# TencentARC/BlobCtrl

Measured on AMD Instinct MI355X. Metric: 512x512_50step_blobctrl_edits_per_sec, higher is better.
Workload: dtype fp16

## Files before the change

blobctrl_amd/_lib.py:

```python
import ctypes as C
import os

_HERE = os.path.dirname(os.path.abspath(__file__))
LIB_PATH = os.environ.get("BLOBCTRL_HIP_LIB") or os.path.join(_HERE, "libblobctrl_hip.so")

A_DENSE, A_CONV3X3 = 0, 1
ACT_NONE, ACT_GELU, ACT_GEGLU, ACT_SILU, ACT_QUICK_GELU = 0, 1, 2, 3, 4
OUT_F16, OUT_F16_T, OUT_F32 = 0, 1, 2
TILE_NAMES = ["auto", "256x128", "128x128_s3", "128x128_s2", "256x64_s2", "256x64_s3", "128x64", "64x64", "halo128x160", "wreg128x160",
              "gw64x128", "gw64x256", "gw64x320", "g256x256"]
TILE_HALO = 8
TILE_WREG = 9
TILE_GW64x128, TILE_GW64x256, TILE_GW64x320 = 10, 11, 12
TILE_G256 = 13
GW_TILES = {TILE_GW64x128: 2, TILE_GW64x256: 4, TILE_GW64x320: 5}


class BcGemm(C.Structure):
    _fields_ = [
        ("A", C.c_void_p), ("A2", C.c_void_p), ("a_mode", C.c_int),
        ("M", C.c_int), ("N", C.c_int), ("K", C.c_int),
        ("lda", C.c_int), ("lda2", C.c_int), ("C1", C.c_int), ("Cin", C.c_int),
        ("Hin", C.c_int), ("Win", C.c_int), ("Hv", C.c_int), ("Wv", C.c_int),
        ("Hout", C.c_int), ("Wout", C.c_int), ("stride", C.c_int), ("conv_nopad_lo", C.c_int),
# ... 130 lines not shown
    "bc_plan_run_timed": (C.c_int, [C.c_void_p, C.c_int, C.c_void_p, C.POINTER(C.c_float)]),
    "bc_plan_run_timed_kernels": (C.c_int, [C.c_void_p, C.c_int, C.c_void_p, C.POINTER(C.c_float), C.POINTER(C.c_float)]),
    "bc_plan_run_marked": (C.c_int, [C.c_void_p, C.c_int, C.POINTER(C.c_void_p), C.c_int, C.POINTER(C.c_int), C.c_int, C.POINTER(C.c_float)]),
    "bc_plan_save": (C.c_int, [C.c_void_p, C.c_char_p, C.c_void_p, C.c_int]),
    "bc_plan_load": (C.c_int, [C.c_char_p, C.POINTER(C.c_void_p)]),
    "bc_plan_buffer": (C.c_int, [C.c_void_p, C.c_char_p, C.POINTER(C.c_void_p), C.POINTER(C.c_longlong)]),
    "bc_graph_begin": (C.c_int, [C.c_void_p]),
    "bc_graph_end": (C.c_int, [C.c_void_p, C.POINTER(C.c_void_p)]),
    "bc_graph_launch": (C.c_int, [C.c_void_p, C.c_void_p]),
    "bc_graph_destroy": (C.c_int, [C.c_void_p]),
    "bc_event_create": (C.c_int, [C.POINTER(C.c_void_p)]),
    "bc_event_create_sync": (C.c_int, [C.POINTER(C.c_void_p)]),
    "bc_stream_wait_event": (C.c_int, [C.c_void_p, C.c_void_p]),
    "bc_event_record": (C.c_int, [C.c_void_p, C.c_void_p]),
    "bc_event_elapsed_ms": (C.c_int, [C.c_void_p, C.c_void_p, C.POINTER(C.c_float)]),
    "bc_event_destroy": (C.c_int, [C.c_void_p]),
}

EXPORTED_SYMBOLS = tuple(_SIGNATURES.keys())

VAE_SIGNATURES = {
    "bc_vae_tile_blend": (C.c_int, [C.c_void_p, C.c_void_p, C.c_void_p, C.c_void_p, C.c_void_p, C.c_int, C.c_int, C.c_int, C.c_int, C.c_int,
                                    C.c_int, C.c_int, C.c_int, C.c_int, C.c_int, C.c_int, C.c_int, C.c_int, C.c_int, C.c_void_p]),
}
VAE_TILE_DECODE, VAE_TILE_ENCODE = 0, 1

REQUEST_SIGNATURES = {
    "bc_assemble_input_requests": (C.c_int, [C.c_void_p, C.c_int, C.c_void_p, C.c_void_p, C.c_void_p, C.c_int, C.c_int, C.c_int,
                                             C.c_int, C.c_int, C.c_int, C.c_int, C.c_void_p, C.c_void_p, C.c_int, C.c_void_p, C.c_void_p]),
    "bc_assemble_input_im2col_requests": (C.c_int, [C.c_void_p, C.c_int, C.c_void_p, C.c_void_p, C.c_int, C.c_int, C.c_int, C.c_int,
                                                    C.c_int, C.c_void_p, C.c_void_p, C.c_int, C.c_void_p, C.c_void_p]),
    "bc_timestep_embedding_rows": (C.c_int, [C.c_void_p, C.c_int, C.c_int, C.c_void_p, C.c_int, C.c_void_p, C.c_void_p]),
    "bc_scheduler_step_requests": (C.c_int, [C.c_void_p, C.c_void_p, C.c_void_p, C.c_void_p, C.c_void_p, C.c_int, C.c_int, C.c_int,
                                             C.c_void_p, C.c_int, C.c_int, C.c_int, C.c_void_p, C.c_int, C.c_void_p]),
}

_ATTN_RELPOS_ARGS = [C.c_void_p] * 4 + [C.c_int] * 11 + [C.c_longlong] * 4 + [C.c_float] + [C.c_void_p] * 3 + [C.c_void_p]
SAM_SIGNATURES = {
    "bc_attention_relpos": (C.c_int, _ATTN_RELPOS_ARGS),
    "bc_window_partition": (C.c_int, [C.c_void_p, C.c_int, C.c_int, C.c_int, C.c_int, C.c_int, C.c_void_p, C.c_void_p]),
    "bc_window_unpartition": (C.c_int, [C.c_void_p, C.c_void_p, C.c_int, C.c_int, C.c_int, C.c_int, C.c_int, C.c_void_p, C.c_void_p]),
    "bc_add_pos": (C.c_int, [C.c_void_p, C.c_void_p, C.c_int, C.c_int, C.c_int, C.c_void_p, C.c_void_p]),
    "bc_add_rows": (C.c_int, [C.c_void_p, C.c_void_p, C.c_int, C.c_int, C.c_int, C.c_void_p, C.c_void_p]),
    "bc_act_rows": (C.c_int, [C.c_void_p, C.c_longlong, C.c_int, C.c_void_p]),
    "bc_bilinear_resize_f32": (C.c_int, [C.c_void_p] + [C.c_int] * 8 + [C.c_float, C.c_void_p, C.c_void_p]),
    "bc_sam_tokens": (C.c_int, [C.c_void_p, C.c_int, C.c_void_p, C.c_void_p, C.c_int, C.c_void_p, C.c_int, C.c_void_p, C.c_void_p, C.c_float,
                                C.c_void_p, C.c_void_p]),
    "bc_sam_masks": (C.c_int, [C.c_void_p, C.c_int, C.c_void_p, C.c_int, C.c_int, C.c_int, C.c_int, C.c_int, C.c_void_p, C.c_void_p]),
}
SAM_BATCH_SIGNATURES = {
    "bc_sam_tokens_batch": (C.c_int, [C.c_void_p, C.c_int, C.c_void_p, C.c_void_p, C.c_int, C.c_int, C.c_void_p, C.c_int, C.c_void_p, C.c_void_p,
                                      C.c_float, C.c_void_p, C.c_void_p]),
    "bc_mask_stats": (C.c_int, [C.c_void_p, C.c_int, C.c_int, C.c_int, C.c_float, C.c_float, C.c_void_p, C.c_void_p, C.c_void_p]),
}
SAM_HOST_SIGNATURES = {"bc_mask_stats_chunks": (C.c_int, [C.c_int, C.c_int])}

_MASK_REMOVE_ARGS = [C.c_void_p, C.c_int, C.c_int, C.c_int, C.c_int, C.c_int, C.c_void_p, C.c_void_p, C.c_void_p]
MASK_SIGNATURES = {
    "bc_mask_label": (C.c_int, [C.c_void_p, C.c_int, C.c_int, C.c_int, C.c_int, C.c_void_p, C.c_void_p]),
    "bc_mask_remove_small": (C.c_int, _MASK_REMOVE_ARGS + [C.c_void_p]),
    "bc_mask_remove_small_phase": (C.c_int, _MASK_REMOVE_ARGS + [C.c_int, C.c_void_p]),
}
MASK_HOLES, MASK_ISLANDS = 0, 1
MASK_REGION_PHASES = 5

EDIT_SIGNATURES = {
    "bc_ellipse_cover": (C.c_int, [C.c_void_p, C.c_int, C.c_int, C.c_int, C.c_void_p, C.c_void_p]),
    "bc_ellipse_paint": (C.c_int, [C.c_void_p, C.c_int, C.c_int, C.c_int, C.c_void_p, C.c_void_p, C.c_int, C.c_void_p]),
    "bc_mask_row_extents": (C.c_int, [C.c_void_p, C.c_int, C.c_int, C.c_int, C.c_void_p, C.c_void_p]),
    "bc_mask_cutout": (C.c_int, [C.c_void_p, C.c_void_p, C.c_void_p, C.c_int, C.c_int, C.c_int, C.c_void_p, C.c_void_p]),
}
EDIT_MAX_DIM = 16384

RESAMPLE_SIGNATURES = {
    "bc_resample_horizontal": (C.c_int, [C.c_void_p, C.c_int, C.c_int, C.c_int, C.c_int, C.c_int, C.c_void_p, C.c_void_p, C.c_int, C.c_int,
                                         C.c_int, C.c_int, C.c_void_p, C.c_void_p]),
    "bc_resample_vertical": (C.c_int, [C.c_void_p, C.c_int, C.c_int, C.c_int, C.c_int, C.c_int, C.c_void_p, C.c_void_p, C.c_int, C.c_int,
                                       C.c_int, C.c_int, C.c_int, C.c_void_p, C.c_void_p, C.c_void_p, C.c_int, C.c_int, C.c_void_p]),
}

_BLUR_ARGS = [C.c_void_p, C.c_int, C.c_int, C.c_int, C.c_int, C.c_int, C.c_int, C.c_void_p, C.c_void_p]
OVERLAY_SIGNATURES = {
    "bc_box_blur3_rows": (C.c_int, _BLUR_ARGS),
    "bc_box_blur3_cols": (C.c_int, _BLUR_ARGS),
    "bc_mask_bounds": (C.c_int, [C.c_void_p, C.c_int, C.c_int, C.c_int, C.c_void_p, C.c_void_p, C.c_void_p]),
    "bc_overlay_composite": (C.c_int, [C.c_void_p, C.c_void_p, C.c_void_p, C.c_int, C.c_int, C.c_int, C.c_int, C.c_int, C.c_int, C.c_int,
                                       C.c_void_p, C.c_void_p]),
}
BLUR_MAX_R = 63

IP_SIGNATURES = {
    "bc_attention_ip": (C.c_int, [C.c_void_p, C.c_void_p, C.c_void_p, C.c_void_p, C.c_int, C.c_int, C.c_int, C.c_int, C.c_int, C.c_int, C.c_int,
                                  C.c_int, C.c_float, C.c_void_p, C.c_void_p]),
}
ATTENTION_IP_MAX_T = 64
IP_PATH_SIGNATURES = {
    "bc_attention_ip_path": (C.c_int, [C.c_int, C.c_int, C.c_int, C.c_int]),
    "bc_attention_ip_with": (C.c_int, [C.c_int] + IP_SIGNATURES["bc_attention_ip"][1]),
}
ATTENTION_IP_SCALAR, ATTENTION_IP_TILES = 0, 1

IP_MASK_SIGNATURES = {
    "bc_attention_ip_masked": (C.c_int, [C.c_void_p, C.c_void_p, C.c_void_p, C.c_void_p, C.c_int, C.c_int, C.c_int, C.c_int, C.c_int, C.c_int,
                                         C.c_int, C.c_int, C.c_int, C.c_float, C.c_void_p, C.c_void_p, C.c_int, C.c_void_p]),
}
IP_MASK_DIRECT_SIGNATURES = {
    "bc_ip_mask_downsample": (C.c_int, [C.c_void_p, C.c_int, C.c_int, C.c_int, C.c_int, C.c_int, C.c_int, C.c_int, C.c_void_p, C.c_int,
                                        C.c_void_p]),
    "bc_attention_ip_masked_path": (C.c_int, [C.c_int] * 5),
    "bc_attention_ip_masked_with": (C.c_int, [C.c_int] + IP_MASK_SIGNATURES["bc_attention_ip_masked"][1]),
}

class BcTinyConvArgs(C.Structure):
    _fields_ = [("x", C.c_void_p), ("w", C.c_void_p), ("bias", C.c_void_p), ("skip", C.c_void_p), ("out", C.c_void_p),
                ("B", C.c_int), ("H", C.c_int), ("W", C.c_int), ("Ci", C.c_int), ("Co", C.c_int),
                ("up", C.c_int), ("relu", C.c_int), ("out_mode", C.c_int)]


TINY_VAE_SIGNATURES = {
    "bc_tiny_conv3x3_flat": (C.c_int, [C.c_void_p] * 5 + [C.c_int] * 8 + [C.c_void_p]),
    "bc_tiny_latents_in": (C.c_int, [C.c_void_p, C.c_int, C.c_int, C.c_int, C.c_void_p, C.c_void_p]),
}
TINY_VAE_DIRECT_SIGNATURES = {"bc_tiny_conv3x3": (C.c_int, [C.POINTER(BcTinyConvArgs), C.c_void_p])}
TINY_OUT_F16, TINY_OUT_IMAGE, TINY_OUT_U8 = 0, 1, 2

PAG_SIGNATURES = {
    "bc_attention_identity": (C.c_int, [C.c_void_p, C.c_void_p, C.c_int, C.c_int, C.c_int, C.c_int, C.c_int, C.c_int, C.c_void_p]),
    "bc_pag_scheduler_step": (C.c_int, [C.c_void_p] * 6 + [C.c_int] * 3 + [C.c_void_p] + [C.c_int] * 3 + [C.c_void_p, C.c_int, C.c_void_p]),
}

OPS = {"bc_gemm": 0, "bc_gn_stats": 1, "bc_gn_finalize": 2, "bc_gn_apply_fused": 3, "bc_gn_apply": 4, "bc_layernorm": 5,
       "bc_attention": 6, "bc_attention_causal": 7, "bc_assemble_input": 8, "bc_timestep_embedding": 9,
       "bc_timestep_embedding_table": 10, "bc_cfg_scheduler_step": 11, "bc_embed_tokens": 12, "bc_softmax_rows": 13,
       "bc_patchify": 14, "bc_add_cls_pos": 15, "bc_silu": 16, "bc_nchw_to_nhwc_f16": 17, "bc_nhwc_to_nchw": 18,
       "bc_gaussian_sample": 19, "bc_rowchain": 22, "bc_assemble_input_im2col": 23, "bc_memset_zero": 24,
       "bc_rowchain_midx": 25, "bc_rowchain_pack_kv": 26, "bc_rowchain_sum": 27, "bc_ctx_fold": 28, "bc_dup_halves": 29,
       "bc_cfg_scheduler_step_noise": 30, "bc_cfg_scheduler_step3": 31,
       "bc_assemble_input_scaled": 32, "bc_assemble_input_im2col_scaled": 33, "bc_scheduler_step_single": 34,
       "bc_timestep_embedding_table_cond": 35, "bc_timestep_embedding_cond": 36, "bc_freeu": 37}
REQUEST_OPS = {"bc_scheduler_step_requests": 38, "bc_assemble_input_requests": 39, "bc_assemble_input_im2col_requests": 40,
               "bc_timestep_embedding_rows": 41}
SAM_OPS = {"bc_attention_relpos": 42, "bc_window_partition": 43, "bc_window_unpartition": 44, "bc_add_pos": 45, "bc_add_rows": 46,
           "bc_act_rows": 47, "bc_bilinear_resize_f32": 48, "bc_sam_tokens": 49, "bc_sam_masks": 50}
SAM_BATCH_OPS = {"bc_sam_tokens_batch": 51, "bc_mask_stats": 52}
IP_OPS = {"bc_attention_ip": 53}
IP_MASK_OPS = {"bc_attention_ip_masked": 55}
_OP_TABLES = (OPS, REQUEST_OPS, SAM_OPS, SAM_BATCH_OPS, IP_OPS)
_OP_TABLES_BEYOND = (IP_MASK_OPS,)
TINY_VAE_OPS = {"bc_tiny_conv3x3_flat": 57, "bc_tiny_latents_in": 58}
_OP_TABLES_TINY_VAE = (TINY_VAE_OPS,)
PAG_OPS = {"bc_attention_identity": 60, "bc_pag_scheduler_step": 61}
_OP_TABLES_PAG = (PAG_OPS,)
OP_SIGNAL, OP_WAIT = 20, 21
CHAIN_IN, CHAIN_MID, CHAIN_OUT, CHAIN_OUT_FF, CHAIN_OUT_TAIL, CHAIN_MIDX, CHAIN_OUT_FFP = 0, 1, 2, 3, 4, 5, 6
GN_TOT_WORDS = 6
_KIND = {C.c_void_p: "p", C.c_int: "i", C.c_float: "f", C.c_longlong: "l", C.c_char_p: "p"}


def op_code(name):
    for table in _OP_TABLES + _OP_TABLES_BEYOND + _OP_TABLES_TINY_VAE + _OP_TABLES_PAG:
        if name in table:
            return table[name]
    raise KeyError(name)


def op_signature(name):
    args = (_SIGNATURES.get(name) or REQUEST_SIGNATURES.get(name) or SAM_SIGNATURES.get(name) or SAM_BATCH_SIGNATURES.get(name) or
            IP_SIGNATURES.get(name) or IP_MASK_SIGNATURES.get(name) or TINY_VAE_SIGNATURES.get(name) or PAG_SIGNATURES[name])[1][:-1]
    return "".join("p" if (a not in _KIND) else _KIND[a] for a in args)


class BcPlanBuffer(C.Structure):
    _fields_ = [("name", C.c_char_p), ("address", C.c_void_p), ("bytes", C.c_longlong), ("host_data", C.c_void_p)]

_lib = None


class BlobCtrlHipError(RuntimeError):
    pass


def load():
    global _lib
    if _lib is not None:
        return _lib
    if not os.path.exists(LIB_PATH):
        raise BlobCtrlHipError(
            f"{LIB_PATH} not found: build it with `python -c 'import __graft_entry__ as g; g.build()'` "
            "(hipcc --offload-arch=gfx950).  blobctrl_amd has no CPU fallback.")
    try:
        import torch
    except ImportError:
        pass
    try:
        lib = C.CDLL(LIB_PATH)
    except OSError as e:
        raise BlobCtrlHipError(f"failed to load {LIB_PATH}: {e}") from e
    for name, (res, args) in list(_SIGNATURES.items()) + list(VAE_SIGNATURES.items()) + list(REQUEST_SIGNATURES.items()) + \
            list(SAM_SIGNATURES.items()) + list(SAM_BATCH_SIGNATURES.items()) + list(SAM_HOST_SIGNATURES.items()) + \
            list(MASK_SIGNATURES.items()) + list(EDIT_SIGNATURES.items()) + list(RESAMPLE_SIGNATURES.items()) + \
            list(IP_SIGNATURES.items()) + list(IP_PATH_SIGNATURES.items()) + list(OVERLAY_SIGNATURES.items()) + \
            list(IP_MASK_SIGNATURES.items()) + list(IP_MASK_DIRECT_SIGNATURES.items()) + list(TINY_VAE_SIGNATURES.items()) + \
            list(TINY_VAE_DIRECT_SIGNATURES.items()) + list(PAG_SIGNATURES.items()):
        fn = getattr(lib, name)
        fn.restype = res
        fn.argtypes = args
    if lib.bc_sizeof_gemm() != C.sizeof(BcGemm):
        raise BlobCtrlHipError(f"BcGemm layout mismatch: C {lib.bc_sizeof_gemm()} vs ctypes {C.sizeof(BcGemm)}")
    _lib = lib
    return lib


def check(rc, what=""):
    if rc != 0:
        msg = load().bc_last_error()
        raise BlobCtrlHipError(f"{what} failed (rc={rc}): {msg.decode() if msg else ''}")
```

blobctrl_amd/csrc/rowchain.hip:

```cpp
#include <stdlib.h>
#include <vector>
#include "bc_common.h"

namespace {

constexpr int RC_BM = 64;
constexpr int RC_NT = 5;
constexpr int RC_HC = 128;
constexpr int RC_RPAD = 20;

template <int C>
struct RCfg {
    static constexpr int NW = C / 80;
    static constexpr int NTH = 64 * NW;
    static constexpr int KS = C / 32;
    static constexpr int NCH = 4 * C / RC_HC;
    static constexpr int HW_ = RC_HC / NW;
    static constexpr int TP = HW_ / 16;
    static constexpr int X_BYTES = KS * 4096;
    static constexpr int S_BYTES = RC_BM * C * 2;
    static constexpr int LDS = X_BYTES + S_BYTES;
    static constexpr int ROWS_PASS = NTH / 8;
    static constexpr int NPASS = RC_BM / ROWS_PASS;
    static constexpr int NKC = C / 64;
    static constexpr int G = RC_NT * KS;
};

struct RowChainArgs {
    int kind, M, rows_per_batch;
    const h16* x;
    const float* affine;
    const unsigned long long* gn_in;
    const float* gn_gamma;
    const float* gn_beta;
    int gn_groups;
    float gn_eps;
    const h16* res;
    const h16* res2;
    const h16* r2;
    int r2_xmin, r2_bmod, out_w;
    const uint4* wstream;
    long long wave_frags;
    const float* vec;
    h16* out0;
    h16* out1;
    h16* out2;
    int ldvt;
    unsigned long long* gn_tot;
    float ln_eps;
    float alpha;
    const float* alpha_dev;
    const int* alpha_idx;
    int alpha_bstride;
    float* part;
    int nsplit;
    unsigned long long* stamps;
};

template <int C>
struct XCfg {
    static constexpr int D = C / 8;
    static constexpr int HPW = 80 / D;
    static constexpr int QKS = D == 40 ? 2 : 3;
    static constexpr int NKT = 5;
    static constexpr int VT = D == 40 ? 3 : 5;
    static constexpr int FR_HEAD = NKT * QKS + VT * 3;
    static constexpr int FR_WAVE = HPW * FR_HEAD;
    static constexpr int P_BYTES = 2 * 4096 + 2048;
};

typedef float f32x4v __attribute__((ext_vector_type(4)));
template <int V> struct IC { static constexpr int value = V; };

__device__ __forceinline__ h16x8 as_h8(uint4 v) { return __builtin_bit_cast(h16x8, v); }

__device__ __forceinline__ void lds_barrier() {
    asm volatile("s_waitcnt lgkmcnt(0)" ::: "memory");
    __builtin_amdgcn_s_barrier();
    asm volatile("" ::: "memory");
}

template <int R>
struct WRing {
    uint4 f[R];
    const uint4* p;
};

template <int R>
__device__ __forceinline__ void ring_fill(WRing<R>& r) {
#pragma unroll
    for (int i = 0; i < R; ++i) r.f[i] = r.p[i * 64];
    r.p += R * 64;
}

template <int NT, int KS, int POS, bool SWAP, int RC_R>
__device__ __forceinline__ void gemm_seg(f32x4v (&acc)[NT][4], WRing<RC_R>& r, const char* xb) {
    h16x8 xq[2][4];
#pragma unroll
    for (int mt = 0; mt < 4; ++mt) xq[0][mt] = *reinterpret_cast<const h16x8*>(xb + mt * 1024);
#pragma unroll
    for (int s = 0; s < KS; ++s) {
        if (s > 0) {
#pragma unroll
            for (int t = 0; t < NT; ++t) r.f[(POS + (s - 1) * NT + t) % RC_R] = r.p[t * 64];
            r.p += NT * 64;
        }
        if (s + 1 < KS) {
#pragma unroll
            for (int mt = 0; mt < 4; ++mt) xq[(s + 1) & 1][mt] = *reinterpret_cast<const h16x8*>(xb + (s + 1) * 4096 + mt * 1024);
        }
        __builtin_amdgcn_sched_barrier(0);
#pragma unroll
        for (int t = 0; t < NT; ++t) {
            const h16x8 w = as_h8(r.f[(POS + s * NT + t) % RC_R]);
#pragma unroll
            for (int mt = 0; mt < 4; ++mt)
                acc[t][mt] = SWAP ? __builtin_amdgcn_mfma_f32_16x16x32_f16(w, xq[s & 1][mt], acc[t][mt], 0, 0, 0)
                                  : __builtin_amdgcn_mfma_f32_16x16x32_f16(xq[s & 1][mt], w, acc[t][mt], 0, 0, 0);
        }
        __builtin_amdgcn_sched_barrier(0);
    }
#pragma unroll
    for (int t = 0; t < NT; ++t) r.f[(POS + (KS - 1) * NT + t) % RC_R] = r.p[t * 64];
    r.p += NT * 64;
    __builtin_amdgcn_sched_barrier(0);
}

template <int NT, int KS, int POS, int RC_R, int JUMP>
__device__ __forceinline__ void gemm_seg_jump(f32x4v (&acc)[NT][4], WRing<RC_R>& r, const uint4* p2, const char* xb) {
    h16x8 xq[2][4];
#pragma unroll
    for (int mt = 0; mt < 4; ++mt) xq[0][mt] = *reinterpret_cast<const h16x8*>(xb + mt * 1024);
#pragma unroll
    for (int s = 0; s < KS; ++s) {
        if (s > 0) {
#pragma unroll
            for (int t = 0; t < NT; ++t)
                r.f[(POS + (s - 1) * NT + t) % RC_R] = (s - 1) * NT + t >= JUMP ? p2[((s - 1) * NT + t - JUMP) * 64] : r.p[t * 64];
            r.p += NT * 64;
        }
        if (s + 1 < KS) {
#pragma unroll
            for (int mt = 0; mt < 4; ++mt) xq[(s + 1) & 1][mt] = *reinterpret_cast<const h16x8*>(xb + (s + 1) * 4096 + mt * 1024);
        }
        __builtin_amdgcn_sched_barrier(0);
#pragma unroll
        for (int t = 0; t < NT; ++t) {
            const h16x8 w = as_h8(r.f[(POS + s * NT + t) % RC_R]);
#pragma unroll
            for (int mt = 0; mt < 4; ++mt) acc[t][mt] = __builtin_amdgcn_mfma_f32_16x16x32_f16(w, xq[s & 1][mt], acc[t][mt], 0, 0, 0);
        }
        __builtin_amdgcn_sched_barrier(0);
    }
#pragma unroll
    for (int t = 0; t < NT; ++t) r.f[(POS + (KS - 1) * NT + t) % RC_R] = (KS - 1) * NT + t >= JUMP ? p2[((KS - 1) * NT + t - JUMP) * 64] : r.p[t * 64];
    r.p = p2 + (NT * KS - JUMP) * 64;
    __builtin_amdgcn_sched_barrier(0);
}

template <int NTV, int TLO, int POS, int RC_R>
__device__ __forceinline__ void pv_seg(f32x4v (&o)[5][4], WRing<RC_R>& r, const char* Pw, int xfo, int m, int q) {
    h16x8 xq[2][4];
#pragma unroll
    for (int mt = 0; mt < 4; ++mt) xq[0][mt] = *reinterpret_cast<const h16x8*>(Pw + mt * 1024 + xfo);
#pragma unroll
    for (int s = 0; s < 3; ++s) {
        if (s > 0) {
#pragma unroll
            for (int t = 0; t < NTV; ++t) r.f[(POS + (s - 1) * NTV + t) % RC_R] = r.p[t * 64];
            r.p += NTV * 64;
        }
        if (s == 0) {
#pragma unroll
            for (int mt = 0; mt < 4; ++mt) xq[1][mt] = *reinterpret_cast<const h16x8*>(Pw + 4096 + mt * 1024 + xfo);
        }
        if (s == 1) {
#pragma unroll
            for (int mt = 0; mt < 4; ++mt) {
                const h16x8 v = *reinterpret_cast<const h16x8*>(Pw + 8192 + (16 * mt + m) * 32 + (q & 1) * 16);
                xq[0][mt] = q < 2 ? v : (h16x8){0, 0, 0, 0, 0, 0, 0, 0};
            }
        }
        __builtin_amdgcn_sched_barrier(0);
#pragma unroll
        for (int t = 0; t < NTV; ++t) {
            const h16x8 w = as_h8(r.f[(POS + s * NTV + t) % RC_R]);
#pragma unroll
            for (int mt = 0; mt < 4; ++mt) o[TLO + t][mt] = __builtin_amdgcn_mfma_f32_16x16x32_f16(w, xq[s & 1][mt], o[TLO + t][mt], 0, 0, 0);
        }
        __builtin_amdgcn_sched_barrier(0);
    }
#pragma unroll
    for (int t = 0; t < NTV; ++t) r.f[(POS + 2 * NTV + t) % RC_R] = r.p[t * 64];
    r.p += NTV * 64;
    __builtin_amdgcn_sched_barrier(0);
}

template <int NT>
__device__ __forceinline__ void zero_acc(f32x4v (&acc)[NT][4]) {
#pragma unroll
    for (int t = 0; t < NT; ++t)
#pragma unroll
        for (int mt = 0; mt < 4; ++mt) acc[t][mt] = (f32x4v){0.f, 0.f, 0.f, 0.f};
}

__device__ __forceinline__ int x_off(int s, int row, int kc) { return s * 4096 + row * 64 + ((kc ^ ((0 - ((row & 15) >> 2)) & 3)) << 4); }
template <int RC_C>
__device__ __forceinline__ int s_off8(int row, int unit) { return row * (RC_C * 2) + ((unit ^ ((row >> 1) & 7)) << 3); }

__device__ __forceinline__ uint4 swap_halves(uint4 d) { return make_uint4(d.z, d.w, d.x, d.y); }

struct CopyMap {
    int row, v8, sw;
    int s_base, x_base;
};

template <int RC_C>
__device__ __forceinline__ CopyMap copy_map(int tid) {
    CopyMap c;
    c.row = tid >> 3;
    c.v8 = tid & 7;
    c.sw = (c.row >> 1) & 7;
    c.s_base = c.row * (RC_C * 2) + ((c.v8 ^ (c.sw >> 1)) << 4);
    c.x_base = x_off(c.v8 >> 2, c.row, c.v8 & 3);
    return c;
}

template <int RC_C>
__device__ __forceinline__ void rows_to_S(const h16* __restrict__ src, char* S, const CopyMap& c, bool masked = false, int pix0 = 0,
                                          int out_w = 1, int xmin = 0) {
    const h16* g = src + (size_t)c.row * RC_C + c.v8 * 8;
#pragma unroll
    for (int j = 0; j < RCfg<RC_C>::NPASS; ++j) {
        const bool zero = masked && ((pix0 + c.row + RCfg<RC_C>::ROWS_PASS * j) % out_w) < xmin;
#pragma unroll
        for (int k = 0; k < RCfg<RC_C>::NKC; ++k) {
            uint4 d = *reinterpret_cast<const uint4*>(g + j * RCfg<RC_C>::ROWS_PASS * RC_C + k * 64);
            if (zero) d = make_uint4(0u, 0u, 0u, 0u);
            if (c.sw & 1) d = swap_halves(d);
            *reinterpret_cast<uint4*>(S + c.s_base + j * RCfg<RC_C>::ROWS_PASS * RC_C * 2 + k * 128) = d;
        }
    }
}

template <int RC_C>
__device__ __forceinline__ void S_to_rows(h16* __restrict__ dst, int ld, const char* S, const CopyMap& c) {
    h16* g = dst + (size_t)c.row * ld + c.v8 * 8;
#pragma unroll
    for (int j = 0; j < RCfg<RC_C>::NPASS; ++j)
#pragma unroll
        for (int k = 0; k < RCfg<RC_C>::NKC; ++k) {
            uint4 d = *reinterpret_cast<const uint4*>(S + c.s_base + j * RCfg<RC_C>::ROWS_PASS * RC_C * 2 + k * 128);
            if (c.sw & 1) d = swap_halves(d);
            *reinterpret_cast<uint4*>(g + (size_t)j * RCfg<RC_C>::ROWS_PASS * ld + k * 64) = d;
        }
}

template <int RC_C>
__device__ __forceinline__ void rows_to_X(const h16* __restrict__ src, char* X, const CopyMap& c, const char* abl, bool ab) {
    const h16* g = src + (size_t)c.row * RC_C + c.v8 * 8;
#pragma unroll
    for (int k = 0; k < RCfg<RC_C>::NKC; ++k) {
        float4 a4[4];
        if (ab) {
#pragma unroll
            for (int j4 = 0; j4 < 4; ++j4) a4[j4] = reinterpret_cast<const float4*>(abl + (c.v8 + 8 * k) * 64)[j4];
        }
#pragma unroll
        for (int j = 0; j < RCfg<RC_C>::NPASS; ++j) {
            uint4 d = *reinterpret_cast<const uint4*>(g + j * RCfg<RC_C>::ROWS_PASS * RC_C + k * 64);
            if (ab) {
                h16* e = reinterpret_cast<h16*>(&d);
#pragma unroll
                for (int j4 = 0; j4 < 4; ++j4) {
                    e[2 * j4] = (h16)fmaf((float)e[2 * j4], a4[j4].x, a4[j4].y);
                    e[2 * j4 + 1] = (h16)fmaf((float)e[2 * j4 + 1], a4[j4].z, a4[j4].w);
                }
            }
            *reinterpret_cast<uint4*>(X + c.x_base + k * 2 * 4096 + j * RCfg<RC_C>::ROWS_PASS * 64) = d;
        }
    }
}

template <int RC_C>
__device__ __forceinline__ void S_to_X(const char* S, char* X, const CopyMap& c) {
#pragma unroll
    for (int j = 0; j < RCfg<RC_C>::NPASS; ++j)
#pragma unroll
        for (int k = 0; k < RCfg<RC_C>::NKC; ++k) {
            uint4 d = *reinterpret_cast<const uint4*>(S + c.s_base + j * RCfg<RC_C>::ROWS_PASS * RC_C * 2 + k * 128);
            if (c.sw & 1) d = swap_halves(d);
            *reinterpret_cast<uint4*>(X + c.x_base + k * 2 * 4096 + j * RCfg<RC_C>::ROWS_PASS * 64) = d;
        }
}

__device__ __forceinline__ h16x4 pack4(const float (&v)[4]) { return (h16x4){(h16)v[0], (h16)v[1], (h16)v[2], (h16)v[3]}; }

template <int RC_C, bool RES>
__device__ __forceinline__ void epi_bias_res(f32x4v (&acc)[RC_NT][4], const float* __restrict__ bias, const char* S, int wave, int m, int q) {
#pragma unroll
    for (int t = 0; t < RC_NT; ++t) {
        const int c0 = 80 * wave + 16 * t + 4 * q;
        const float4 b = bias ? *reinterpret_cast<const float4*>(bias + c0) : make_float4(0.f, 0.f, 0.f, 0.f);
#pragma unroll
        for (int mt = 0; mt < 4; ++mt) {
            acc[t][mt][0] += b.x; acc[t][mt][1] += b.y; acc[t][mt][2] += b.z; acc[t][mt][3] += b.w;
            if (RES) {
                const h16x4 rr = *reinterpret_cast<const h16x4*>(S + s_off8<RC_C>(16 * mt + m, c0 >> 2));
#pragma unroll
                for (int r = 0; r < 4; ++r) acc[t][mt][r] += (float)rr[r];
            }
        }
    }
}

template <int RC_C>
__device__ __forceinline__ void acc_to_S(const f32x4v (&acc)[RC_NT][4], char* S, int wave, int m, int q, float scale = 1.0f) {
#pragma unroll
    for (int t = 0; t < RC_NT; ++t) {
        const int c0 = 80 * wave + 16 * t + 4 * q;
#pragma unroll
        for (int mt = 0; mt < 4; ++mt) {
            const float v[4] = {acc[t][mt][0] * scale, acc[t][mt][1] * scale, acc[t][mt][2] * scale, acc[t][mt][3] * scale};
            *reinterpret_cast<h16x4*>(S + s_off8<RC_C>(16 * mt + m, c0 >> 2)) = pack4(v);
        }
    }
}

__device__ __forceinline__ void acc_to_X(const f32x4v (&acc)[RC_NT][4], char* X, int wave, int m, int q) {
#pragma unroll
    for (int t = 0; t < RC_NT; ++t) {
        const int c0 = 80 * wave + 16 * t + 4 * q;
#pragma unroll
        for (int mt = 0; mt < 4; ++mt) {
            const float v[4] = {acc[t][mt][0], acc[t][mt][1], acc[t][mt][2], acc[t][mt][3]};
            *reinterpret_cast<h16x4*>(X + x_off(c0 >> 5, 16 * mt + m, (c0 & 31) >> 3) + ((c0 >> 2) & 1) * 8) = pack4(v);
        }
    }
}

template <int RC_C>
__device__ __forceinline__ void layernorm_to_X(const f32x4v (&acc)[RC_NT][4], const float* __restrict__ gb, float eps, char* X, int wave,
                                               int m, int q) {
    constexpr int NW = RCfg<RC_C>::NW;
    float* st = reinterpret_cast<float*>(X);
    float mean[4], rstd[4];
    auto row_total = [&](const float* p) {
        float4 v = *reinterpret_cast<const float4*>(p);
        float t = (v.x + v.y) + (v.z + v.w);
        if (NW == 8) {
            v = *reinterpret_cast<const float4*>(p + 4);
            t += (v.x + v.y) + (v.z + v.w);
        }
        return t;
    };
    lds_barrier();
#pragma unroll
    for (int mt = 0; mt < 4; ++mt) {
        float s = 0.f;
#pragma unroll
        for (int t = 0; t < RC_NT; ++t) s += (acc[t][mt][0] + acc[t][mt][1]) + (acc[t][mt][2] + acc[t][mt][3]);
        s += __shfl_xor(s, 16);
        s += __shfl_xor(s, 32);
        if (q == 0) st[(16 * mt + m) * NW + wave] = s;
    }
    lds_barrier();
#pragma unroll
    for (int mt = 0; mt < 4; ++mt) {
        mean[mt] = row_total(st + (16 * mt + m) * NW) * (1.0f / RC_C);
        float s = 0.f;
#pragma unroll
        for (int t = 0; t < RC_NT; ++t)
#pragma unroll
            for (int r = 0; r < 4; ++r) {
                const float d = acc[t][mt][r] - mean[mt];
                s = fmaf(d, d, s);
            }
        s += __shfl_xor(s, 16);
        s += __shfl_xor(s, 32);
        if (q == 0) st[64 * NW + (16 * mt + m) * NW + wave] = s;
    }
    lds_barrier();
#pragma unroll
    for (int mt = 0; mt < 4; ++mt) rstd[mt] = __builtin_amdgcn_rsqf(row_total(st + 64 * NW + (16 * mt + m) * NW) * (1.0f / RC_C) + eps);
    lds_barrier();
#pragma unroll
    for (int t = 0; t < RC_NT; ++t) {
        const int c0 = 80 * wave + 16 * t + 4 * q;
        const float4 g = *reinterpret_cast<const float4*>(gb + c0);
        const float4 b = *reinterpret_cast<const float4*>(gb + RC_C + c0);
#pragma unroll
        for (int mt = 0; mt < 4; ++mt) {
            const float v[4] = {fmaf((acc[t][mt][0] - mean[mt]) * rstd[mt], g.x, b.x), fmaf((acc[t][mt][1] - mean[mt]) * rstd[mt], g.y, b.y),
                                fmaf((acc[t][mt][2] - mean[mt]) * rstd[mt], g.z, b.z), fmaf((acc[t][mt][3] - mean[mt]) * rstd[mt], g.w, b.w)};
            *reinterpret_cast<h16x4*>(X + x_off(c0 >> 5, 16 * mt + m, (c0 & 31) >> 3) + ((c0 >> 2) & 1) * 8) = pack4(v);
        }
    }
}

template <int RC_C>
__device__ __forceinline__ void gn_partials_from_S(const char* S, char* scratch, unsigned long long* __restrict__ dst, int tid, int spread) {
    float* const sc = reinterpret_cast<float*>(scratch);
    if (tid < RC_C / 2) {
        float s0 = 0.f, s1 = 0.f, q0 = 0.f, q1 = 0.f;
        const int unit = tid >> 1, half = tid & 1;
#pragma unroll 8
        for (int row = 0; row < RC_BM; ++row) {
            const h16x2 v = *reinterpret_cast<const h16x2*>(S + s_off8<RC_C>(row, unit) + half * 4);
            const float a = (float)v[0], b = (float)v[1];
            s0 += a; q0 = fmaf(a, a, q0);
            s1 += b; q1 = fmaf(b, b, q1);
        }
        *reinterpret_cast<float4*>(sc + 4 * tid) = make_float4(s0, q0, s1, q1);
    }
    lds_barrier();
    for (int c = tid; c < RC_C; c += (int)blockDim.x)
        bc_gn_tot_add_slot(dst, c, 0, RC_C, bc_gn_cg(RC_C), spread, [&](int k) { return make_float2(sc[2 * k], sc[2 * k + 1]); });
    lds_barrier();
}

template <int RC_C, int KIND, bool BLOB>
__global__ __launch_bounds__(RCfg<RC_C>::NTH, 2) void rowchain_kernel(const RowChainArgs a) {
    using CF = RCfg<RC_C>;
    constexpr int RC_KS = CF::KS, RC_NCH = CF::NCH;
    extern __shared__ __attribute__((aligned(16))) char smem[];
    char* X = smem;
    char* S = smem + CF::X_BYTES;
    const int tid = threadIdx.x;
    const int lane = tid & 63;
    const int wave = __builtin_amdgcn_readfirstlane(tid >> 6);
    const int m = lane & 15, q = lane >> 4;
    constexpr bool FFP = KIND == BC_CHAIN_OUT_FFP;
    constexpr bool FF = KIND == BC_CHAIN_OUT_FF || FFP, TAIL = KIND == BC_CHAIN_OUT_TAIL;
    const int wg = bc_xcd_remap(blockIdx.x, gridDim.x);
    const int nrb = a.M / RC_BM;
    const int z = FFP ? wg / nrb : (FF ? wg % a.nsplit : 0);
    const int m0 = (FFP ? wg % nrb : (FF ? wg / a.nsplit : wg)) * RC_BM;
    const int b = m0 / a.rows_per_batch;
    const int pix0 = m0 - b * a.rows_per_batch;
    const int xfo = m * 64 + ((q ^ ((0 - (m >> 2)) & 3)) << 4);
    const float* vec = a.vec;
    const CopyMap cm = copy_map<RC_C>(tid);
    unsigned long long* const stamps = a.stamps;
    unsigned long long acc_t[3] = {0, 0, 0};
    auto stamp = [&](int i) {
        if (stamps && tid == 0) stamps[(size_t)blockIdx.x * 16 + i] = __builtin_amdgcn_s_memtime();
    };
    stamp(0);

    if (KIND == BC_CHAIN_IN && a.gn_in) {
        constexpr int NTH = CF::NTH, PER = (RC_C + NTH - 1) / NTH;
        float* abl = reinterpret_cast<float*>(S);
        double* scr = reinterpret_cast<double*>(S + RC_C * 8);
        float* stat = reinterpret_cast<float*>(S + RC_C * 24);
        float gp[PER], bp_[PER];
#pragma unroll
        for (int j = 0; j < PER; ++j) {
            const int c = tid + NTH * j;
            gp[j] = c < RC_C ? a.gn_gamma[c] : 0.f;
            bp_[j] = c < RC_C ? a.gn_beta[c] : 0.f;
        }
#pragma unroll
        for (int j = 0; j < PER; ++j) {
            const int c = tid + NTH * j;
            if (c < RC_C) {
                double s_, q_;
                bc_gn_tot_read(a.gn_in + ((size_t)b * RC_C + c) * BC_GN_TOT_WORDS, s_, q_);
                scr[c * 2] = s_;
                scr[c * 2 + 1] = q_;
            }
        }
        __syncthreads();
        const int cpg = RC_C / a.gn_groups, sub = tid & 7;
        for (int gi = tid >> 3; gi < a.gn_groups; gi += NTH / 8) {
            double s_ = 0.0, q_ = 0.0;
            for (int cj = sub; cj < cpg; cj += 8) {
                s_ += scr[(gi * cpg + cj) * 2];
                q_ += scr[(gi * cpg + cj) * 2 + 1];
            }
#pragma unroll
            for (int o = 4; o > 0; o >>= 1) {
                s_ += __shfl_xor(s_, o);
                q_ += __shfl_xor(q_, o);
            }
            const double n = (double)a.rows_per_batch * cpg;
            const double mean = s_ / n;
            double var = q_ / n - mean * mean;
            if (var < 0.0) var = 0.0;
            if (sub == 0) {
                stat[gi * 2] = (float)mean;
                stat[gi * 2 + 1] = (float)(1.0 / sqrt(var + (double)a.gn_eps));
            }
        }
        __syncthreads();
#pragma unroll
        for (int j = 0; j < PER; ++j) {
            const int c = tid + NTH * j;
            if (c < RC_C) {
                const int gi = c / cpg;
                const float av = stat[gi * 2 + 1] * gp[j];
                abl[c * 2] = av;
                abl[c * 2 + 1] = bp_[j] - stat[gi * 2] * av;
            }
        }
        __syncthreads();
    } else if (KIND == BC_CHAIN_IN && a.affine) {
        const float4* src4 = reinterpret_cast<const float4*>(a.affine + (size_t)b * RC_C * 2);
        for (int i = tid; i < RC_C / 2; i += CF::NTH) reinterpret_cast<float4*>(S)[i] = src4[i];
        __syncthreads();
    }
    constexpr bool FFLOOP = KIND == BC_CHAIN_OUT || FF;
    constexpr bool MIDX = KIND == BC_CHAIN_MIDX;
    constexpr int RC_R = RC_C == 320 ? (FFLOOP ? 15 : (KIND == BC_CHAIN_IN ? 13 : (MIDX ? 12 : 16)))
                                     : (FFLOOP ? 10 : (KIND == BC_CHAIN_IN ? 12 : (MIDX ? 8 : 12)));
    static_assert(RC_R <= RC_RPAD, "stream padding");
    WRing<RC_R> ring;
    ring.p = a.wstream + ((size_t)z * CF::NW + wave) * a.wave_frags * 64 + lane;
    ring_fill(ring);

    f32x4v acc[RC_NT][4];
    zero_acc(acc);

    if (KIND == BC_CHAIN_IN) {
        rows_to_X<RC_C>(a.x + (size_t)m0 * RC_C, X, cm, S, a.gn_in != nullptr || a.affine != nullptr);
        lds_barrier();
        stamp(1);
        gemm_seg<RC_NT, RC_KS, 0, true>(acc, ring, X + xfo);
        stamp(2);
        epi_bias_res<RC_C, false>(acc, vec, S, wave, m, q);
        layernorm_to_X<RC_C>(acc, vec + RC_C, a.ln_eps, X, wave, m, q);
        stamp(3);
        acc_to_S<RC_C>(acc, S, wave, m, q);
        lds_barrier();
        S_to_rows<RC_C>(a.out0 + (size_t)m0 * RC_C, RC_C, S, cm);
        zero_acc(acc);
        gemm_seg<RC_NT, RC_KS, (RC_NT * RC_KS) % RC_R, true>(acc, ring, X + xfo);
        lds_barrier();
        acc_to_S<RC_C>(acc, S, wave, m, q);
        lds_barrier();
        S_to_rows<RC_C>(a.out1 + (size_t)m0 * 2 * RC_C, 2 * RC_C, S, cm);
        zero_acc(acc);
        gemm_seg<RC_NT, RC_KS, (2 * RC_NT * RC_KS) % RC_R, true>(acc, ring, X + xfo);
        lds_barrier();
        acc_to_S<RC_C>(acc, S, wave, m, q);
        lds_barrier();
        S_to_rows<RC_C>(a.out1 + (size_t)m0 * 2 * RC_C + RC_C, 2 * RC_C, S, cm);
        zero_acc(acc);
        gemm_seg<RC_NT, RC_KS, (3 * RC_NT * RC_KS) % RC_R, false>(acc, ring, X + xfo);
        lds_barrier();
#pragma unroll
        for (int t = 0; t < RC_NT; ++t) {
            const int ch = 80 * wave + 16 * t + m;
#pragma unroll
            for (int mt = 0; mt < 4; ++mt) {
                const float v[4] = {acc[t][mt][0], acc[t][mt][1], acc[t][mt][2], acc[t][mt][3]};
                *reinterpret_cast<h16x4*>(S + ch * 128 + (((4 * mt + q) ^ (ch & 15)) << 3)) = pack4(v);
            }
        }
        lds_barrier();
        {
            const int ch0 = tid >> 3, part = tid & 7, sw = ch0 & 15;
            h16* vt = a.out2 + ((size_t)b * RC_C + ch0) * a.ldvt + pix0 + part * 8;
            const char* sp = S + ch0 * 128 + ((part ^ (sw >> 1)) << 4);
#pragma unroll
            for (int i = 0; i < RC_C / CF::ROWS_PASS; ++i) {
                uint4 d = *reinterpret_cast<const uint4*>(sp + i * CF::ROWS_PASS * 128);
                if (sw & 1) d = swap_halves(d);
                *reinterpret_cast<uint4*>(vt + (size_t)i * CF::ROWS_PASS * a.ldvt) = d;
            }
        }
        stamp(4);
        return;
    }

    if (!TAIL) {
        rows_to_X<RC_C>(a.x + (size_t)m0 * RC_C, X, cm, S, false);
        rows_to_S<RC_C>(a.res + (size_t)m0 * RC_C, S, cm);
        lds_barrier();
        stamp(1);
        gemm_seg<RC_NT, RC_KS, 0, true>(acc, ring, X + xfo);
        stamp(2);
        epi_bias_res<RC_C, true>(acc, vec, S, wave, m, q);
    }

    if (KIND == BC_CHAIN_MID) {
        layernorm_to_X<RC_C>(acc, vec + RC_C, a.ln_eps, X, wave, m, q);
        acc_to_S<RC_C>(acc, S, wave, m, q);
        lds_barrier();
        S_to_rows<RC_C>(a.out0 + (size_t)m0 * RC_C, RC_C, S, cm);
        zero_acc(acc);
        gemm_seg<RC_NT, RC_KS, (RC_NT * RC_KS) % RC_R, true>(acc, ring, X + xfo);
        lds_barrier();
        acc_to_S<RC_C>(acc, S, wave, m, q);
        lds_barrier();
        S_to_rows<RC_C>(a.out1 + (size_t)m0 * RC_C, RC_C, S, cm);
        stamp(4);
        return;
    }
    if constexpr (MIDX) {
        using XC = XCfg<RC_C>;
        constexpr int G = RC_NT * RC_KS;
        layernorm_to_X<RC_C>(acc, vec + RC_C, a.ln_eps, X, wave, m, q);
        acc_to_S<RC_C>(acc, S, wave, m, q);
        lds_barrier();
        S_to_rows<RC_C>(a.out0 + (size_t)m0 * RC_C, RC_C, S, cm);
        zero_acc(acc);
        gemm_seg_jump<RC_NT, RC_KS, G % RC_R, RC_R, G - RC_R>(
            acc, ring, reinterpret_cast<const uint4*>(a.res2) + ((size_t)b * CF::NW + wave) * (XC::FR_WAVE + RC_RPAD) * 64 + lane, X + xfo);
        lds_barrier();
        acc_to_X(acc, X, wave, m, q);
        f32x4v o[RC_NT][4];
        zero_acc(o);
        char* Pw = S + wave * XC::P_BYTES;
        const float csc = a.alpha * 1.4426950408889634f;
        const int T = a.r2_xmin;
        auto head = [&](auto hc) {
            constexpr int hh = decltype(hc)::value;
            constexpr int POS_K = (2 * G + hh * XC::FR_HEAD) % RC_R, POS_V = (POS_K + XC::NKT * XC::QKS) % RC_R;
            constexpr int TLO = XC::D == 40 && hh == 1 ? 2 : 0;
            const int s0 = (80 * wave + XC::D * hh) >> 5;
            zero_acc(acc);
            gemm_seg<XC::NKT, XC::QKS, POS_K, true, RC_R>(acc, ring, X + s0 * 4096 + xfo);
#pragma unroll
            for (int mt = 0; mt < 4; ++mt) {
                float mx = -3.0e38f;
#pragma unroll
                for (int t = 0; t < XC::NKT; ++t)
#pragma unroll
                    for (int r = 0; r < 4; ++r)
                        if (16 * t + 4 * q + r < T) mx = fmaxf(mx, acc[t][mt][r]);
                mx = fmaxf(mx, __shfl_xor(mx, 16));
                mx = fmaxf(mx, __shfl_xor(mx, 32));
                float sum = 0.f;
#pragma unroll
                for (int t = 0; t < XC::NKT; ++t)
#pragma unroll
                    for (int r = 0; r < 4; ++r) {
                        const float e = 16 * t + 4 * q + r < T ? __builtin_amdgcn_exp2f((acc[t][mt][r] - mx) * csc) : 0.f;
                        acc[t][mt][r] = e;
                        sum += e;
                    }
                sum += __shfl_xor(sum, 16);
                sum += __shfl_xor(sum, 32);
                const float inv = __builtin_amdgcn_rcpf(sum);
#pragma unroll
                for (int t = 0; t < XC::NKT; ++t) {
                    const float v[4] = {acc[t][mt][0] * inv, acc[t][mt][1] * inv, acc[t][mt][2] * inv, acc[t][mt][3] * inv};
                    char* dst = t < 4 ? Pw + x_off(t >> 1, 16 * mt + m, 2 * (t & 1) + (q >> 1)) + (q & 1) * 8 : Pw + 8192 + (16 * mt + m) * 32 + q * 8;
                    *reinterpret_cast<h16x4*>(dst) = pack4(v);
                }
            }
            pv_seg<XC::VT, TLO, POS_V, RC_R>(o, ring, Pw, xfo, m, q);
        };
        head(IC<0>{});
        if constexpr (XC::HPW == 2) head(IC<1>{});
        lds_barrier();
        int tid2 = threadIdx.x;
        asm volatile("" : "+v"(tid2));
        const int m2 = tid2 & 15, q2 = (tid2 & 63) >> 4;
        acc_to_S<RC_C>(o, S, wave, m2, q2);
        lds_barrier();
        S_to_rows<RC_C>(a.out1 + (size_t)m0 * RC_C, RC_C, S, copy_map<RC_C>(tid2));
        stamp(4);
        return;
    }

    if (!TAIL) {
    layernorm_to_X<RC_C>(acc, vec + RC_C, a.ln_eps, X, wave, m, q);
    lds_barrier();
    stamp(3);
    if (FF && z != 0) zero_acc(acc);
    const int c_lo = FF ? z * (RC_NCH / a.nsplit) : 0, c_hi = FF ? c_lo + RC_NCH / a.nsplit : RC_NCH;
    {
        const float* b1 = vec + 3 * RC_C;
        constexpr int POS_FF = (RC_NT * RC_KS) % RC_R;
        constexpr int TP = CF::TP, HPW = CF::HW_;
        static_assert(!FFLOOP || (TP * 2 * RC_KS + RC_NT * (RC_HC / 32)) % RC_R == 0,
                      "a feed-forward chunk must consume a whole number of rings");
        for (int c = c_lo; c < c_hi; ++c) {
            char* P = S + (c & 1) * 16384;
            const float* bb = b1 + (c * CF::NW + wave) * (2 * HPW) + 4 * q;
            float4 bvg[2 * TP];
#pragma unroll
            for (int i = 0; i < 2 * TP; ++i) bvg[i] = *reinterpret_cast<const float4*>(bb + 16 * i);
#pragma unroll
            for (int tp = 0; tp < TP; ++tp) {
                f32x4v a1[2][4];
                zero_acc(a1);
                const unsigned long long ta = stamps ? __builtin_amdgcn_s_memtime() : 0;
                if (tp == 0) gemm_seg<2, RC_KS, POS_FF, true>(a1, ring, X + xfo);
                else gemm_seg<2, RC_KS, (POS_FF + 2 * RC_KS) % RC_R, true>(a1, ring, X + xfo);
                const unsigned long long tb = stamps ? __builtin_amdgcn_s_memtime() : 0;
                acc_t[0] += tb - ta;
                const float4 bv = bvg[2 * tp], bg = bvg[2 * tp + 1];
                const int hc0 = HPW * wave + 16 * tp + 4 * q;
#pragma unroll
                for (int mt = 0; mt < 4; ++mt) {
                    const f32x2 g01 = bc_gelu_f2((f32x2){a1[1][mt][0], a1[1][mt][1]} + (f32x2){bg.x, bg.y});
                    const f32x2 g23 = bc_gelu_f2((f32x2){a1[1][mt][2], a1[1][mt][3]} + (f32x2){bg.z, bg.w});
                    const f32x2 v01 = ((f32x2){a1[0][mt][0], a1[0][mt][1]} + (f32x2){bv.x, bv.y}) * g01;
                    const f32x2 v23 = ((f32x2){a1[0][mt][2], a1[0][mt][3]} + (f32x2){bv.z, bv.w}) * g23;
                    const float v[4] = {v01.x, v01.y, v23.x, v23.y};
                    *reinterpret_cast<h16x4*>(P + x_off(hc0 >> 5, 16 * mt + m, (hc0 & 31) >> 3) + ((hc0 >> 2) & 1) * 8) = pack4(v);
                }
                if (stamps) acc_t[1] += __builtin_amdgcn_s_memtime() - tb;
            }
            lds_barrier();
            const unsigned long long tc = stamps ? __builtin_amdgcn_s_memtime() : 0;
            gemm_seg<RC_NT, RC_HC / 32, (POS_FF + TP * 2 * RC_KS) % RC_R, true>(acc, ring, P + xfo);
            if (stamps) acc_t[2] += __builtin_amdgcn_s_memtime() - tc;
        }
    }
    }
    stamp(4);
    if (stamps && tid == 0) {
        stamps[(size_t)blockIdx.x * 16 + 8] = acc_t[0];
        stamps[(size_t)blockIdx.x * 16 + 9] = acc_t[1];
        stamps[(size_t)blockIdx.x * 16 + 10] = acc_t[2];
    }
    if (KIND == BC_CHAIN_OUT_FF) {
        float* dst = a.part + ((size_t)z * a.M + m0) * RC_C + 80 * wave + 4 * q;
#pragma unroll
        for (int t = 0; t < RC_NT; ++t)
#pragma unroll
            for (int mt = 0; mt < 4; ++mt) *reinterpret_cast<f32x4v*>(dst + (size_t)(16 * mt + m) * RC_C + 16 * t) = acc[t][mt];
        stamp(7);
        return;
    }
    if (TAIL) {
        const float* src = a.part + (size_t)m0 * RC_C + 80 * wave + 4 * q;
        for (int zz = 0; zz < a.nsplit; ++zz)
#pragma unroll
            for (int t = 0; t < RC_NT; ++t)
#pragma unroll
                for (int mt = 0; mt < 4; ++mt)
                    acc[t][mt] += *reinterpret_cast<const f32x4v*>(src + ((size_t)zz * a.M + 16 * mt + m) * RC_C + 16 * t);
    }
    int m_ = m, q_ = q, xfo_ = xfo;
    CopyMap cm_ = cm;
    asm volatile("" : "+v"(m_), "+v"(q_), "+v"(xfo_), "+v"(cm_.row), "+v"(cm_.v8), "+v"(cm_.sw), "+v"(cm_.s_base), "+v"(cm_.x_base));
#define m m_
#define q q_
#define xfo xfo_
#define cm cm_
    const bool first = !FFP || z == 0;
    if (first) epi_bias_res<RC_C, false>(acc, vec + 3 * RC_C + 8 * RC_C, S, wave, m, q);
    lds_barrier();
    acc_to_X(acc, X, wave, m, q);
    if (first) rows_to_S<RC_C>(a.res2 + (size_t)m0 * RC_C, S, cm);
    lds_barrier();
    zero_acc(acc);
    constexpr int POS_PO = TAIL ? 0 : (RC_NT * RC_KS) % RC_R;
    stamp(5);
    gemm_seg<RC_NT, RC_KS, POS_PO, true>(acc, ring, X + xfo);
    stamp(6);
    const float* bpo = vec + 3 * RC_C + 8 * RC_C + RC_C;
    if (first) epi_bias_res<RC_C, true>(acc, bpo, S, wave, m, q);
    if (a.r2 && first) {
        const bool any = ((pix0 % a.out_w) + RC_BM > a.r2_xmin) || (pix0 % a.out_w) + RC_BM > a.out_w;
        if (any) {
            lds_barrier();
            rows_to_S<RC_C>(a.r2 + ((size_t)(b % a.r2_bmod) * a.rows_per_batch + pix0) * RC_C, S, cm, true, pix0, a.out_w, a.r2_xmin);
            lds_barrier();
            epi_bias_res<RC_C, true>(acc, nullptr, S, wave, m, q);
        }
    }
    lds_barrier();
    acc_to_S<RC_C>(acc, S, wave, m, q);
    lds_barrier();
    h16* const p16 = reinterpret_cast<h16*>(a.part);
    S_to_rows<RC_C>(FFP ? p16 + ((size_t)z * a.M + m0) * RC_C : a.out0 + (size_t)m0 * RC_C, RC_C, S, cm);
    if (!FFP && a.gn_tot) gn_partials_from_S<RC_C>(S, X, a.gn_tot + (size_t)b * RC_C * BC_GN_TOT_WORDS, tid, m0 / RC_BM);
    stamp(7);
    if (BLOB) {
        S_to_X<RC_C>(S, X, cm);
        lds_barrier();
        zero_acc(acc);
        gemm_seg<RC_NT, RC_KS, (POS_PO + RC_NT * RC_KS) % RC_R, true>(acc, ring, X + xfo);
        if (first) epi_bias_res<RC_C, false>(acc, bpo + RC_C, S, wave, m, q);
        float alpha = a.alpha;
        if (a.alpha_dev) alpha *= a.alpha_dev[(a.alpha_idx ? *a.alpha_idx : 0) * (a.alpha_bstride > 0 ? a.alpha_bstride : 1) + (a.alpha_bstride > 0 ? b : 0)];
        lds_barrier();
        acc_to_S<RC_C>(acc, S, wave, m, q, alpha);
        lds_barrier();
        S_to_rows<RC_C>(FFP ? p16 + ((size_t)(a.nsplit + z) * a.M + m0) * RC_C : a.out1 + (size_t)m0 * RC_C, RC_C, S, cm);
    }
#undef m
#undef q
#undef xfo
#undef cm
}

struct RcStampReport {
    hipStream_t stream; size_t n; unsigned long long* buf; int kind;
    ~RcStampReport() {
        if (!buf) return;
        if (hipStreamSynchronize(stream) != hipSuccess) return;
        std::vector<unsigned long long> h(n * 16);
        if (hipMemcpy(h.data(), buf, n * 16 * sizeof(unsigned long long), hipMemcpyDeviceToHost) != hipSuccess) return;
        double d[8] = {0}, ff[3] = {0};
        unsigned long long t0 = ~0ull, t1 = 0;
        const int last = kind == BC_CHAIN_OUT ? 7 : 4;
        for (size_t i = 0; i < n; ++i) {
            for (int k = 0; k < last; ++k) d[k] += (double)(h[i * 16 + k + 1] - h[i * 16 + k]);
            for (int k = 0; k < 3; ++k) ff[k] += (double)h[i * 16 + 8 + k];
            t0 = std::min(t0, h[i * 16]);
            t1 = std::max(t1, h[i * 16 + last]);
        }
        if (kind == BC_CHAIN_OUT)
            fprintf(stderr, "[rowchain stamps out] wgs=%zu | avg ticks: prologue %.0f, to_out gemm %.0f, epilogue+LN %.0f, ff loop %.0f (ff1 gemms %.0f, "
                    "geglu %.0f, ff2 gemms %.0f), h3 + x staging %.0f, proj_out gemm %.0f, epilogue+stores %.0f | first entry -> last exit %llu ticks\n",
                    n, d[0] / n, d[1] / n, d[2] / n, d[3] / n, ff[0] / n, ff[1] / n, ff[2] / n, d[4] / n, d[5] / n, d[6] / n, t1 - t0);
        else
            fprintf(stderr, "[rowchain stamps %s] wgs=%zu | avg ticks: prologue %.0f, first gemm %.0f, epilogue+LN %.0f, rest %.0f | first entry -> last "
                    "exit %llu ticks\n", kind == BC_CHAIN_IN ? "in" : kind == BC_CHAIN_MIDX ? "midx" : "mid", n, d[0] / n, d[1] / n, d[2] / n, d[3] / n, t1 - t0);
    }
};

template <int RC_C, int KIND, bool BLOB>
int launch_chain(const RowChainArgs& a_in, hipStream_t stream) {
    using CF = RCfg<RC_C>;
    RowChainArgs a = a_in;
    static const bool want_stamps = getenv("BC_RC_STAMPS") != nullptr;
    static unsigned long long* stamp_buf = nullptr;
    const size_t nwg = (size_t)a.M / RC_BM;
    a.stamps = nullptr;
    if (want_stamps && nwg <= 8192) {
        if (!stamp_buf) BC_CHECK_HIP(hipMalloc(reinterpret_cast<void**>(&stamp_buf), 8192 * 16 * sizeof(unsigned long long)));
        BC_CHECK_HIP(hipMemsetAsync(stamp_buf, 0, nwg * 16 * sizeof(unsigned long long), stream));
        a.stamps = stamp_buf;
    }
    RcStampReport report{stream, nwg, a.stamps, KIND};
    static std::atomic<unsigned long long> lds_set{0};
    BC_CHECK_HIP(bc_set_max_lds(lds_set, reinterpret_cast<const void*>(&rowchain_kernel<RC_C, KIND, BLOB>), CF::LDS));
    hipLaunchKernelGGL((rowchain_kernel<RC_C, KIND, BLOB>), dim3(a.M / RC_BM * (KIND == BC_CHAIN_OUT_FF || KIND == BC_CHAIN_OUT_FFP ? a.nsplit : 1)), dim3(CF::NTH), CF::LDS, stream, a);
    BC_CHECK_LAUNCH();
    return 0;
}

#ifndef BC_ROWCHAIN_MIDX_TU
constexpr int SUM_ROWS = 64;
template <int RC_C>
__global__ __launch_bounds__(640) void rowchain_sum_kernel(const h16* __restrict__ part, int nsplit, int M, int rows_per_batch, h16* __restrict__ out0,
                                                           unsigned long long* __restrict__ gn_tot, h16* __restrict__ out1) {
    constexpr int NC = RC_C / 8, RL = 640 / NC, RPT = SUM_ROWS / RL;
    __shared__ float red[RL][NC][16];
    const int tid = threadIdx.x, cg = tid % NC, rl = tid / NC;
    const int m0 = blockIdx.x * SUM_ROWS;
    float s[8], q[8];
#pragma unroll
    for (int j = 0; j < 8; ++j) s[j] = q[j] = 0.f;
#pragma unroll
    for (int i = 0; i < RPT; ++i) {
        const size_t off = (size_t)(m0 + rl + RL * i) * RC_C + cg * 8;
#pragma unroll
        for (int o = 0; o < 2; ++o) {
            if (o == 1 && !out1) break;
            float v[8];
#pragma unroll
            for (int j = 0; j < 8; ++j) v[j] = 0.f;
            for (int z = 0; z < nsplit; ++z) {
                const h16x8 d = *reinterpret_cast<const h16x8*>(part + ((size_t)(o * nsplit + z) * M) * RC_C + off);
#pragma unroll
                for (int j = 0; j < 8; ++j) v[j] += (float)d[j];
            }
            h16x8 r;
#pragma unroll
            for (int j = 0; j < 8; ++j) r[j] = (h16)v[j];
            *reinterpret_cast<h16x8*>((o ? out1 : out0) + off) = r;
            if (o == 0) {
#pragma unroll
                for (int j = 0; j < 8; ++j) {
                    const float f = (float)r[j];
                    s[j] += f;
                    q[j] = fmaf(f, f, q[j]);
                }
            }
        }
    }
    if (gn_tot) {
#pragma unroll
        for (int j = 0; j < 8; ++j) {
            red[rl][cg][j] = s[j];
            red[rl][cg][8 + j] = q[j];
        }
        __syncthreads();
        const int b = m0 / rows_per_batch;
        if (tid < RC_C)
            bc_gn_tot_add_slot(gn_tot + (size_t)b * RC_C * BC_GN_TOT_WORDS, tid, 0, RC_C, bc_gn_cg(RC_C), (int)blockIdx.x, [&](int k) {
                float ss = 0.f, qq = 0.f;
#pragma unroll
                for (int r2 = 0; r2 < RL; ++r2) {
                    ss += red[r2][k >> 3][k & 7];
                    qq += red[r2][k >> 3][8 + (k & 7)];
                }
                return make_float2(ss, qq);
            });
    }
}

template <int RC_C>
long long stream_frags(int kind, int blobnet, int nsplit) {
    using CF = RCfg<RC_C>;
    const long long g = CF::G;
    const long long per_chunk = CF::TP * 2 * CF::KS + RC_NT * (RC_HC / 32);
    long long n = 0;
    if (kind == BC_CHAIN_IN) n = 4 * g;
    else if (kind == BC_CHAIN_MID || kind == BC_CHAIN_MIDX) n = 2 * g;
    else if (kind == BC_CHAIN_OUT) n = 2 * g + CF::NCH * per_chunk + (blobnet ? g : 0);
    else if (kind == BC_CHAIN_OUT_FF && nsplit > 0 && CF::NCH % nsplit == 0) n = g + CF::NCH / nsplit * per_chunk;
    else if (kind == BC_CHAIN_OUT_FFP && nsplit > 0 && CF::NCH % nsplit == 0) n = 2 * g + CF::NCH / nsplit * per_chunk + (blobnet ? g : 0);
    else if (kind == BC_CHAIN_OUT_TAIL) n = g + (blobnet ? g : 0);
    else return -1;
    return n + RC_RPAD;
}

template <int RC_C>
int dispatch_chain(int kind, bool blob, const RowChainArgs& a, hipStream_t s) {
    switch (kind) {
        case BC_CHAIN_IN: return launch_chain<RC_C, BC_CHAIN_IN, false>(a, s);
        case BC_CHAIN_MID: return launch_chain<RC_C, BC_CHAIN_MID, false>(a, s);
        case BC_CHAIN_OUT_FF: return launch_chain<RC_C, BC_CHAIN_OUT_FF, false>(a, s);
        case BC_CHAIN_OUT_TAIL: return blob ? launch_chain<RC_C, BC_CHAIN_OUT_TAIL, true>(a, s) : launch_chain<RC_C, BC_CHAIN_OUT_TAIL, false>(a, s);
        case BC_CHAIN_OUT_FFP: return blob ? launch_chain<RC_C, BC_CHAIN_OUT_FFP, true>(a, s) : launch_chain<RC_C, BC_CHAIN_OUT_FFP, false>(a, s);
        default: return blob ? launch_chain<RC_C, BC_CHAIN_OUT, true>(a, s) : launch_chain<RC_C, BC_CHAIN_OUT, false>(a, s);
    }
}

}

extern "C" int bc_rowchain_supported(int channels, int M, int rows_per_batch) {
    return (channels == 320 || channels == 640) && M > 0 && rows_per_batch > 0 && M % rows_per_batch == 0 && rows_per_batch % RC_BM == 0;
}

extern "C" long long bc_rowchain_stream_frags(int channels, int kind, int blobnet, int nsplit) {
    if (channels == 320) return stream_frags<320>(kind, blobnet, nsplit);
    if (channels == 640) return stream_frags<640>(kind, blobnet, nsplit);
    return -1;
}

extern "C" int bc_rowchain(int kind, int channels, int M, int rows_per_batch, const bc_half* x, const float* affine,
                           const unsigned long long* gn_in, const float* gn_gamma, const float* gn_beta, int gn_groups, float gn_eps, const bc_half* res,
                           const bc_half* res2, const bc_half* r2, int r2_xmin, int r2_bmod, int out_w, const bc_half* wstream,
                           const float* vec, bc_half* out0, bc_half* out1, bc_half* out2, int ldvt, unsigned long long* gn_tot, float ln_eps,
                           float alpha, const float* alpha_dev, const int* alpha_idx, int alpha_bstride, float* part, int nsplit,
                           bc_stream stream) {
    BC_CHECK_ARG(bc_rowchain_supported(channels, M, rows_per_batch), "bc_rowchain: needs 320 or 640 channels, M %% rows_per_batch == 0 and "
                 "rows_per_batch %% %d == 0 (channels=%d M=%d rows_per_batch=%d)", RC_BM, channels, M, rows_per_batch);
    BC_CHECK_ARG((kind >= BC_CHAIN_IN && kind <= BC_CHAIN_OUT_TAIL) || kind == BC_CHAIN_OUT_FFP, "bc_rowchain: unknown kind %d", kind);
    BC_CHECK_ARG(wstream && vec && (x || kind == BC_CHAIN_OUT_TAIL) && (out0 || kind == BC_CHAIN_OUT_FF || kind == BC_CHAIN_OUT_FFP),
                 "bc_rowchain: null pointer");
    const bool blob = (kind == BC_CHAIN_OUT || kind == BC_CHAIN_OUT_TAIL || kind == BC_CHAIN_OUT_FFP) && out1 != nullptr;
    if (kind == BC_CHAIN_OUT_FF || kind == BC_CHAIN_OUT_TAIL || kind == BC_CHAIN_OUT_FFP)
        BC_CHECK_ARG(part && nsplit >= 1 && (4 * channels / 128) % nsplit == 0, "bc_rowchain(OUT_FF / OUT_TAIL): needs the partial-sum buffer and nsplit "
                     "dividing the %d hidden chunks (nsplit=%d)", 4 * channels / 128, nsplit);
    RowChainArgs a;
    a.kind = kind; a.M = M; a.rows_per_batch = rows_per_batch;
    a.x = reinterpret_cast<const h16*>(x); a.affine = affine;
    a.gn_in = kind == BC_CHAIN_IN ? gn_in : nullptr; a.gn_gamma = gn_gamma; a.gn_beta = gn_beta; a.gn_groups = gn_groups; a.gn_eps = gn_eps;
    if (a.gn_in)
        BC_CHECK_ARG(gn_gamma && gn_beta && gn_groups > 0 && channels % gn_groups == 0 && channels / gn_groups >= 1 && !affine,
                     "bc_rowchain(IN): the in-kernel GroupNorm finalize needs gamma, beta, groups | channels (and no affine table)");
    a.res = reinterpret_cast<const h16*>(res); a.res2 = reinterpret_cast<const h16*>(res2);
    a.r2 = reinterpret_cast<const h16*>(r2); a.r2_xmin = r2_xmin; a.r2_bmod = r2_bmod > 0 ? r2_bmod : 1; a.out_w = out_w > 0 ? out_w : 1;
    a.wstream = reinterpret_cast<const uint4*>(wstream);
    a.wave_frags = bc_rowchain_stream_frags(channels, kind, blob ? 1 : 0, nsplit);
    a.part = part; a.nsplit = nsplit > 0 ? nsplit : 1;
    a.vec = vec;
    a.out0 = reinterpret_cast<h16*>(out0); a.out1 = reinterpret_cast<h16*>(out1); a.out2 = reinterpret_cast<h16*>(out2);
    a.ldvt = ldvt; a.gn_tot = gn_tot; a.ln_eps = ln_eps;
    a.alpha = alpha; a.alpha_dev = alpha_dev; a.alpha_idx = alpha_idx; a.alpha_bstride = alpha_bstride;
    a.stamps = nullptr;
    hipStream_t s = reinterpret_cast<hipStream_t>(stream);
    if (kind == BC_CHAIN_IN)
        BC_CHECK_ARG(out1 && out2 && ldvt >= rows_per_batch && ldvt % 8 == 0, "bc_rowchain(IN): needs out1 (q|k), out2 (V^T) and ldvt >= rows_per_batch, ldvt %% 8 == 0");
    if (kind == BC_CHAIN_MID) BC_CHECK_ARG(res && out1, "bc_rowchain(MID): needs res and out1");
    if (kind == BC_CHAIN_OUT_FF) BC_CHECK_ARG(res, "bc_rowchain(OUT_FF): needs res");
    if (kind == BC_CHAIN_OUT_FFP) {
        BC_CHECK_ARG(res && res2 && !gn_tot, "bc_rowchain(OUT_FFP): needs res and res2; the statistics totals belong to bc_rowchain_sum");
        BC_CHECK_ARG(!r2 || (out_w > 0 && rows_per_batch % out_w == 0), "bc_rowchain(OUT_FFP): r2 needs out_w dividing rows_per_batch");
    }
    if (kind == BC_CHAIN_OUT || kind == BC_CHAIN_OUT_TAIL) {
        BC_CHECK_ARG((res || kind == BC_CHAIN_OUT_TAIL) && res2, "bc_rowchain(OUT / OUT_TAIL): needs res and res2");
        BC_CHECK_ARG(!r2 || (out_w > 0 && rows_per_batch % out_w == 0), "bc_rowchain(OUT): r2 needs out_w dividing rows_per_batch");
    }
    return channels == 320 ? dispatch_chain<320>(kind, blob, a, s) : dispatch_chain<640>(kind, blob, a, s);
}

extern "C" int bc_rowchain_sum(int channels, int M, int rows_per_batch, const bc_half* part, int nsplit, bc_half* out0, unsigned long long* gn_tot,
                               bc_half* out1, bc_stream stream) {
    BC_CHECK_ARG(bc_rowchain_supported(channels, M, rows_per_batch), "bc_rowchain_sum: needs 320 or 640 channels, M %% rows_per_batch == 0 and "
                 "rows_per_batch %% %d == 0 (channels=%d M=%d rows_per_batch=%d)", RC_BM, channels, M, rows_per_batch);
    BC_CHECK_ARG(part && out0 && nsplit >= 1 && nsplit <= 40, "bc_rowchain_sum: null pointer or nsplit = %d outside 1..40", nsplit);
    hipStream_t s = reinterpret_cast<hipStream_t>(stream);
    if (channels == 320)
        hipLaunchKernelGGL(rowchain_sum_kernel<320>, dim3(M / SUM_ROWS), dim3(640), 0, s, reinterpret_cast<const h16*>(part), nsplit, M, rows_per_batch,
                           reinterpret_cast<h16*>(out0), gn_tot, reinterpret_cast<h16*>(out1));
    else
        hipLaunchKernelGGL(rowchain_sum_kernel<640>, dim3(M / SUM_ROWS), dim3(640), 0, s, reinterpret_cast<const h16*>(part), nsplit, M, rows_per_batch,
                           reinterpret_cast<h16*>(out0), gn_tot, reinterpret_cast<h16*>(out1));
    BC_CHECK_LAUNCH();
    return 0;
}

#else
}

namespace {

template <int RC_C>
__global__ void rowchain_pack_kv_kernel(const h16* __restrict__ k, int ldk, const h16* __restrict__ vt, int ldvt, int B, int T, long long kvf,
                                        uint4* __restrict__ out) {
    using XC = XCfg<RC_C>;
    constexpr int NW = RCfg<RC_C>::NW;
    const long long idx = (long long)blockIdx.x * blockDim.x + threadIdx.x;
    if (idx >= (long long)B * NW * kvf * 64) return;
    const int lane = (int)(idx & 63);
    const long long fi = idx >> 6;
    const int f = (int)(fi % kvf), w = (int)((fi / kvf) % NW), b = (int)(fi / (kvf * NW));
    h16 v[8];
#pragma unroll
    for (int j = 0; j < 8; ++j) v[j] = (h16)0.f;
    if (f < XC::FR_WAVE) {
        const int hh = f / XC::FR_HEAD, g = f % XC::FR_HEAD;
        const int c_h = 80 * w + XC::D * hh;
        if (g < XC::NKT * XC::QKS) {
            const int ks = g / XC::NKT, t = g % XC::NKT;
            const int key = 16 * t + (lane & 15), ch0 = 32 * ((c_h >> 5) + ks) + 8 * (lane >> 4);
#pragma unroll
            for (int j = 0; j < 8; ++j)
                if (key < T && ch0 + j >= c_h && ch0 + j < c_h + XC::D) v[j] = k[((size_t)b * T + key) * ldk + ch0 + j];
        } else {
            const int g2 = g - XC::NKT * XC::QKS;
            const int ks = g2 / XC::VT, tv = g2 % XC::VT;
            const int tlo = XC::D == 40 && hh == 1 ? 2 : 0;
            const int ch = 80 * w + 16 * (tlo + tv) + (lane & 15), key0 = 32 * ks + 8 * (lane >> 4);
            if (ch >= c_h && ch < c_h + XC::D) {
#pragma unroll
                for (int j = 0; j < 8; ++j)
                    if (key0 + j < T) v[j] = vt[((size_t)b * RC_C + ch) * ldvt + key0 + j];
            }
        }
    }
    out[idx] = *reinterpret_cast<const uint4*>(v);
}

}

extern "C" long long bc_rowchain_kv_frags(int channels) {
    if (channels == 320) return XCfg<320>::FR_WAVE + RC_RPAD;
    if (channels == 640) return XCfg<640>::FR_WAVE + RC_RPAD;
    return -1;
}

extern "C" int bc_rowchain_pack_kv(const bc_half* k, int ldk, const bc_half* vt, int ldvt, int B, int T, int channels, bc_half* out, bc_stream stream) {
    BC_CHECK_ARG((channels == 320 || channels == 640) && k && vt && out && B > 0 && T > 0 && T <= 80 && ldk >= channels && ldvt >= T,
                 "bc_rowchain_pack_kv: needs 320 or 640 channels (8 heads), 1 <= T <= 80 context tokens, ldk >= channels, ldvt >= T (channels=%d T=%d)", channels, T);
    const long long kvf = bc_rowchain_kv_frags(channels);
    const long long total = (long long)B * (channels / 80) * kvf * 64;
    hipStream_t s = reinterpret_cast<hipStream_t>(stream);
    if (channels == 320)
        hipLaunchKernelGGL(rowchain_pack_kv_kernel<320>, dim3(bc_ceil_div(total, 256)), dim3(256), 0, s, reinterpret_cast<const h16*>(k), ldk,
                           reinterpret_cast<const h16*>(vt), ldvt, B, T, kvf, reinterpret_cast<uint4*>(out));
    else
        hipLaunchKernelGGL(rowchain_pack_kv_kernel<640>, dim3(bc_ceil_div(total, 256)), dim3(256), 0, s, reinterpret_cast<const h16*>(k), ldk,
                           reinterpret_cast<const h16*>(vt), ldvt, B, T, kvf, reinterpret_cast<uint4*>(out));
    BC_CHECK_LAUNCH();
    return 0;
}

extern "C" int bc_rowchain_midx(int channels, int M, int rows_per_batch, const bc_half* x, const bc_half* res, const bc_half* wstream, const float* vec,
                                const bc_half* kvstream, int n_ctx, float attn_scale, bc_half* out0, bc_half* out1, float ln_eps, bc_stream stream) {
    BC_CHECK_ARG(bc_rowchain_supported(channels, M, rows_per_batch), "bc_rowchain_midx: needs 320 or 640 channels, M %% rows_per_batch == 0 and "
                 "rows_per_batch %% %d == 0 (channels=%d M=%d rows_per_batch=%d)", RC_BM, channels, M, rows_per_batch);
    BC_CHECK_ARG(x && res && wstream && vec && kvstream && out0 && out1 && n_ctx >= 1 && n_ctx <= 80 && attn_scale > 0.f,
                 "bc_rowchain_midx: null pointer, or n_ctx = %d outside 1..80", n_ctx);
    RowChainArgs a = {};
    a.kind = BC_CHAIN_MIDX; a.M = M; a.rows_per_batch = rows_per_batch;
    a.x = reinterpret_cast<const h16*>(x); a.res = reinterpret_cast<const h16*>(res);
    a.r2_bmod = 1; a.out_w = 1; a.nsplit = 1;
    a.wstream = reinterpret_cast<const uint4*>(wstream);
    a.wave_frags = bc_rowchain_stream_frags(channels, BC_CHAIN_MID, 0, 1);
    a.vec = vec;
    a.res2 = reinterpret_cast<const h16*>(kvstream); a.r2_xmin = n_ctx; a.alpha = attn_scale;
    a.out0 = reinterpret_cast<h16*>(out0); a.out1 = reinterpret_cast<h16*>(out1);
    a.ln_eps = ln_eps;
    hipStream_t s = reinterpret_cast<hipStream_t>(stream);
    return channels == 320 ? launch_chain<320, BC_CHAIN_MIDX, false>(a, s) : launch_chain<640, BC_CHAIN_MIDX, false>(a, s);
}
#endif
```

blobctrl_amd/engine.py:

```python
import os
from dataclasses import dataclass
from typing import List, Optional, Tuple

import torch

from . import _lib
from .launch import Recorder
from .options import opt
from .weights import PackedTrunk, pad8


@dataclass
class TrunkConfig:
    in_channels: int
    block_out_channels: Tuple[int, ...] = (320, 640, 1280, 1280)
    layers_per_block: int = 2
    num_heads: int = 8
    norm_num_groups: int = 32
    cross_attention_dim: Optional[int] = 768
    out_channels: int = 4
    is_blobnet: bool = False
    time_cond_proj_dim: Optional[int] = None


# ... 187 lines not shown
        return out

    def gn_conv(self, x: Act, x2: Optional[Act], norm, eps, wname, Cout, **kw):
        pw = self.pw
        C2 = x2.C if x2 is not None else 0
        if self.halo_ok(x.C + C2, C2 and x.C, Cout, x.H, x.W):
            requests = self.B if self.cfg.is_blobnet else max(1, self.B // 2)
            if opt("gn_pass_min_requests") and requests >= opt("gn_pass_min_requests") and x.C + C2 >= opt("gn_pass_min_cin") and opt("wreg"):
                return self.conv3x3(self.groupnorm(x, x2, norm, eps, True), wname, Cout, halo=True, **kw)
            gn = dict(x1=x.t, C1=x.C, x2=x2.t if x2 is not None else None, C2=C2, B=self.B, HW=x.H * x.W, G=self.G, eps=eps,
                      gamma=pw.f[norm + ".weight"], beta=pw.f[norm + ".bias"])
            return self.conv3x3(x, wname, Cout, x2=x2, affine=(gn, _lib.ACT_SILU), halo=True, **kw)
        assert kw.get("sc") is None
        return self.conv3x3(self.groupnorm(x, x2, norm, eps, True), wname, Cout, **kw)

    def sc_fold_ok(self, Cmid, Cout, H, W, Cs, S1):
        return opt("sc_fold") and opt("wreg") and self.halo_ok(Cmid, 0, Cout, H, W) and \
            bool(self.rec.lib.bc_conv_wreg_sc_eligible(Cmid, Cout, H, W, Cs, S1, 0))

    def groupnorm(self, x: Act, x2: Optional[Act], name, eps, silu):
        pw = self.pw
        C2 = x2.C if x2 is not None else 0
        out = self.rec.groupnorm(x.t, x.C, x2.t if x2 is not None else None, C2, self.B, x.H * x.W, self.G, eps,
                                 pw.f[name + ".weight"], pw.f[name + ".bias"], silu)
        return Act(out, x.C + C2, x.H, x.W)

    def freeu(self, h: Act, sk: Act, stage: int):
        assert (h.H, h.W) == (sk.H, sk.W)
        rec = self.rec
        cache = rec.__dict__.setdefault("_freeu_basis", {})
        if (h.H, h.W) not in cache:
            cache[(h.H, h.W)] = rec.register(freeu_basis(h.H, h.W).to(torch.float32).to(rec.device))
            rec.keep.append(cache[(h.H, h.W)])
        ht, st = rec.freeu(h.t, h.C, sk.t, sk.C, self.B, h.H, h.W, self.freeu_params, stage, cache[(h.H, h.W)])
        return Act(ht, h.C, h.H, h.W), Act(st, sk.C, sk.H, sk.W)

    def resnet(self, p, x: Act, skip: Optional[Act], Cout, r2=None, out=None):
        pw = self.pw
        Cin = x.C + (skip.C if skip is not None else 0)
        off, n = pw.temb_slices[p]
        assert n == Cout
        rowvec = (self.tproj.data_ptr() + off * 2, pw.temb_total) + self.tproj_table
        h = self.gn_conv(x, skip, p + "norm1", 1e-5, p + "conv1", Cout, rowvec=rowvec)
        M = self.B * x.H * x.W
        if (p + "conv_shortcut.weight") in pw.h and self.sc_fold_ok(Cout, Cout, x.H, x.W, Cin, x.C if skip is not None else 0):
            return self.gn_conv(h, None, p + "norm2", 1e-5, p + "conv2", Cout, sc=(p + "conv_shortcut", x, skip), r2=r2,
                                **({"out": out} if out is not None else {}))
        if (p + "conv_shortcut.weight") in pw.h:
            kw = {}
            if skip is not None:
                kw.update(A2=skip.t, C1=x.C, lda=x.C, lda2=skip.C)
            gw = self.gw_tile(M, Cout, Cin, x.C if skip is not None else 0) if Cout >= 1280 else 0
            if gw:
                w, _, b = pw.gw(p + "conv_shortcut.weight", gw, bias=p + "conv_shortcut.bias")
                sc_t = self.rec.empty(M, Cout)
                self.rec.gemm(A=x.t, W=w, M=M, N=Cout, K=Cin, out=sc_t, bias=b, tile_cfg=gw, kind="conv1x1", **kw)
                sc = Act(sc_t, Cout, x.H, x.W)
            else:
                sc = Act(self.dense(x.t, M, Cin, p + "conv_shortcut", Cout, kind="conv1x1", **kw), Cout, x.H, x.W)
        else:
            assert skip is None and Cin == Cout
            sc = x
        return self.gn_conv(h, None, p + "norm2", 1e-5, p + "conv2", Cout, R=sc, r2=r2, **({"out": out} if out is not None else {}))

    def rowchain_ok(self, Cc, M, HW, p=""):
        if not opt("rowchain") or not self.rec.lib.bc_rowchain_supported(Cc, M, HW):
            return False
        min_blocks = {320: 1, 640: opt("rowchain_min_blocks_640")}[Cc]
        if Cc == 640 and self.cfg.is_blobnet and p.startswith("up_blocks"):
            min_blocks = opt("rowchain_min_blocks_640_blob_up")
        return M // 64 >= min_blocks

    def rowchain_ff_split(self, Cc, M):
        blocks = M // 64
        if Cc == 640:
            dflt = 4 if self.rowchain_ffp() else 2
            if self.cfg.is_blobnet and opt("ff_split_640_blob"):
                return opt("ff_split_640_blob") if blocks <= 64 else 1
            return (opt("ff_split_640") or dflt) if blocks <= 64 else 1
        return opt("ff_split_320") if blocks <= 128 else 1

    def rowchain_ffp(self):
        if not opt("ffp"):
            return False
        return not self.cfg.is_blobnet or opt("ffp_blob")

    def transformer_rowchain(self, p, x: Act, r2=None, zero=None, fan_out=None):
        from .weights import pack_rowchain
        rec, pw, B = self.rec, self.pw, self.B
        Cc, HW = x.C, x.H * x.W
        M = B * HW
        d = Cc // self.heads
        scale = d ** -0.5
        bp = p + "transformer_blocks.0."
        cache = pw.__dict__.setdefault("_rowchain", {})

        def packed(kind, zname=None, nsplit=1):
            key = (p, kind, zname, nsplit)
            if key not in cache:
                cache[key] = pack_rowchain(pw, p, kind, zname, nsplit)
            return cache[key]
        if opt("gn_finalize_launch"):
            gnkw = dict(affine=rec.gn_affine(x.t, Cc, None, 0, B, HW, self.G, 1e-6, pw.f[p + "norm.weight"], pw.f[p + "norm.bias"]))
        else:
            gnkw = dict(gn_in=(rec.gn_sources(x.t, Cc, None, 0, B, HW, self.G)[0], pw.f[p + "norm.weight"], pw.f[p + "norm.bias"], self.G, 1e-6))
        ldvt = (HW + 63) // 64 * 64
        vt = rec.zeros(B, Cc, ldvt)
        mult = 2 if fan_out is not None else 1
        h0_all, a_all = rec.empty(mult * M, Cc), rec.empty(mult * M, Cc)
        h0, qk = h0_all[:M], rec.empty(M, 2 * Cc)
        w, v = packed(_lib.CHAIN_IN)
        rec.rowchain(_lib.CHAIN_IN, Cc, M, HW, x.t, w, v, h0, out1=qk, out2=vt, ldvt=ldvt, **gnkw)
        a = a_all[:M]
        self.self_attention(p, qk, vt, a, B, d, HW, Cc, ldvt, scale)
        if fan_out is not None:
            x_full, extra = fan_out
            half = M * Cc * 2
            rec.dup_halves([(h0_all, half), (a_all, half), (x_full, half)] + list(extra))
            B, M = 2 * B, 2 * M
            h0, a, x = h0_all, a_all, Act(x_full, Cc, x.H, x.W)
        h = h0
        if pw.has_cross:
            h1 = rec.empty(M, Cc)
            w, v = packed(_lib.CHAIN_MID)
            ck, cvt, T, ldc_vt = self.ctx_kv[bp]
            kvs = self.ctx_kvs.get(bp)
            if kvs is not None:
                a2 = rec.empty(M, Cc)
                rec.rowchain_midx(Cc, M, HW, a, w, v, kvs, T, self.heads, scale, h1, a2, res=h0)
                a = a2
            else:
                q2 = rec.empty(M, Cc)
                rec.rowchain(_lib.CHAIN_MID, Cc, M, HW, a, w, v, h1, out1=q2, res=h0)
                a = rec.empty(M, Cc)
                rec.attention(q2, ck, cvt, a, B, self.heads, d, HW, T, Cc, Cc, ldc_vt, Cc, HW * Cc, T * Cc, Cc * ldc_vt, HW * Cc, scale)
                self.attention_ip(bp, q2, a, B, HW, Cc, d, scale)
            h = h1
        out = rec.empty(M, Cc)
        part = rec.new_tot(B, Cc)
        kw = {}
        r2kw = self._r2(r2, x.H, x.W)
        if r2kw:
            assert r2kw["ldr2"] == Cc
            kw.update(r2=r2kw["R2"], r2_xmin=r2kw["r2_xmin"], r2_bmod=r2kw["r2_bmod"], out_w=r2kw["out_w"])
        res_out = None
        if zero is not None:
            zname, alpha, alpha_dev, alpha_idx, alpha_bstride = zero
            res_out = rec.empty(M, Cc)
            kw.update(out1=res_out, alpha=alpha, alpha_dev=alpha_dev, alpha_idx=alpha_idx, alpha_bstride=alpha_bstride)
        zname = zero[0] if zero is not None else None
        nsplit = self.rowchain_ff_split(Cc, M)
        if nsplit > 1 and self.rowchain_ffp():
            pp = rec.empty((2 if zero is not None else 1) * nsplit, M, Cc)
            w, v = packed(_lib.CHAIN_OUT_FFP, zname, nsplit)
            kw2 = {k: v_ for k, v_ in kw.items() if k != "out1"}
            rec.rowchain(_lib.CHAIN_OUT_FFP, Cc, M, HW, a, w, v, None, out1=res_out, res=h, res2=x.t, part=pp, nsplit=nsplit, **kw2)
            rec.rowchain_sum(Cc, M, HW, pp, nsplit, out, gn_tot=part, out1=res_out)
        elif nsplit > 1:
            ffp = rec.empty(nsplit, M, Cc, dtype=torch.float32)
            w, v = packed(_lib.CHAIN_OUT_FF, zname, nsplit)
            rec.rowchain(_lib.CHAIN_OUT_FF, Cc, M, HW, a, w, v, None, res=h, part=ffp, nsplit=nsplit)
            w, v = packed(_lib.CHAIN_OUT_TAIL, zname)
            rec.rowchain(_lib.CHAIN_OUT_TAIL, Cc, M, HW, None, w, v, out, res2=x.t, gn_tot=part, part=ffp, nsplit=nsplit, **kw)
        else:
            w, v = packed(_lib.CHAIN_OUT, zname)
            rec.rowchain(_lib.CHAIN_OUT, Cc, M, HW, a, w, v, out, res=h, res2=x.t, gn_tot=part, **kw)
        rec.tots[out.data_ptr()] = part
        return Act(out, Cc, x.H, x.W), res_out

    def self_attention(self, p, qk, vt, a, B, d, HW, Cc, ldvt, scale):
        rec = self.rec
        n_ptb = self.pag_images if p in self.pag_layers else 0
        assert 0 <= n_ptb < B and (n_ptb == 0 or B == self.B), "PAG: the perturbed images are the last ones of the whole UNet batch"
        rec.attention(qk, qk, vt, a, B - n_ptb, self.heads, d, HW, HW, 2 * Cc, 2 * Cc, ldvt, Cc, HW * 2 * Cc, HW * 2 * Cc, Cc * ldvt, HW * Cc,
                      scale, q_off=0, k_off=Cc)
        if n_ptb:
            rec.attention_identity(vt, a, B, B - n_ptb, HW, Cc, ldvt, Cc)

    def attention_ip(self, bp, q, a, B, HW, Cc, d, scale):
        for K_ip, V_ip, T_ip, w, *rest in self.ip_kv.get(bp, ()):
            ad = rest[0] if rest else None
            if ad is not None and ad.masked:
                mask = ad.mask_buffer(self.rec, HW)
                self.rec.attention_ip_masked(q, K_ip, V_ip, a, B, HW, self.heads, d, ad.n_images, T_ip // ad.n_images, Cc, Cc, Cc, scale, w,
                                             mask, mask.shape[1])
            else:
                self.rec.attention_ip(q, K_ip, V_ip, a, B, HW, self.heads, d, T_ip, Cc, Cc, Cc, scale, w)

    def gw_tile(self, M, N, K, C1=0, prefer=None):
        if not opt("gw") or M > opt("gw_maxm"):
            return 0
        order = prefer or (_lib.TILE_GW64x128,)
        for cfg in order:
            if self.rec.lib.bc_gemm_wreg_eligible(M, N, K, C1, cfg):
                return cfg
        return 0

    def ctx_fold_ok(self, Cc, T):
        return (self.B <= opt("ctx_fold_maxb") and Cc % 320 == 0 and Cc not in (320, 640) and self.heads == 8 and T <= 80 and (Cc // self.heads) % 8 == 0 and Cc // self.heads <= 160
                and opt("ctx_fold") and opt("gw"))

    def transformer_gw(self, p, x: Act, r2=None):
        rec, pw, B = self.rec, self.pw, self.B
        Cc, HW = x.C, x.H * x.W
        M = B * HW
        d = Cc // self.heads
        scale = d ** -0.5
        bp = p + "transformer_blocks.0."
        G128, G256, G320 = _lib.TILE_GW64x128, _lib.TILE_GW64x256, _lib.TILE_GW64x320

        def proj(a_t, wname, N, K, cfg, ln=None, bias=True, extra=(), **kw):
            for c in (cfg, G128, G320, G256):
                bn = 64 * _lib.GW_TILES[c]
                if N % bn == 0 and kw.get("n_t0", 0) % bn == 0 and rec.lib.bc_gemm_wreg_eligible(M, N, K, kw.get("C1", 0), c):
                    cfg = c
                    break
            w, cs, b = pw.gw(wname + ".weight", cfg, ln=ln, bias=(wname + ".bias") if bias else None, extra=extra)
            n_out = N // 2 if kw.get("act") == _lib.ACT_GEGLU else N
            out = kw.pop("out", None)
            if out is None:
                out = rec.empty(M, kw.get("n_t0") or n_out)
            rec.gemm(A=a_t, W=w, M=M, N=N, K=K, out=out, bias=b, tile_cfg=cfg, ln_colsum=cs, **kw)
            return out
        gn = dict(x1=x.t, C1=Cc, B=B, HW=HW, G=self.G, eps=1e-6, gamma=pw.f[p + "norm.weight"], beta=pw.f[p + "norm.bias"])
        h = proj(x.t, p + "proj_in", Cc, Cc, G128, kind="conv1x1", a_gn=gn, rows_per_batch=HW)
        ldvt = (HW + 63) // 64 * 64
        vt = rec.zeros(B, Cc, ldvt)
        qk = proj(h, bp + "attn1.to_qk", 3 * Cc, Cc, G128, ln=bp + "norm1", bias=False, extra=(bp + "attn1.to_v.weight",), C_t=vt, ldc_t=ldvt,
                  n_t0=2 * Cc, rows_per_batch=HW, kind="qkv")
        a = rec.empty(M, Cc)
        self.self_attention(p, qk, vt, a, B, d, HW, Cc, ldvt, scale)
        h = proj(a, bp + "attn1.to_out.0", Cc, Cc, G128, R=h, ldr=Cc, kind="attn_out")
        folded = self.ctx_folded.get(bp) if pw.has_cross else None
        if folded is not None and rec.lib.bc_gemm_wreg_eligible(M, 128 * self.heads, Cc, 0, G128) and rec.lib.bc_gemm_wreg_eligible(M, Cc, 80 * self.heads, 0, G128):
            wqk, cs, qb, vwo = folded
            T = self.ctx_kv[bp][2]
            N, Np = 128 * self.heads, 80 * self.heads
            pr = rec.empty(M, Np)
            rec.gemm(A=h, W=wqk, M=M, N=N, K=Cc, out=pr, ldc=Np, bias=qb, tile_cfg=G128, ln_colsum=cs, rows_per_batch=HW, w_bstride=wqk.shape[1],
                     vec_bstride=N, sm_group=128, sm_valid=T, sm_keep=80, kind="xattn")
            out = rec.empty(M, Cc)
            rec.gemm(A=pr, W=vwo, M=M, N=Cc, K=Np, out=out, bias=pw.f[bp + "attn2.to_out.0.bias"], tile_cfg=G128, R=h, ldr=Cc, rows_per_batch=HW,
                     w_bstride=vwo.shape[1], kind="xattn")
            h = out
        elif pw.has_cross:
            q = proj(h, bp + "attn2.to_q", Cc, Cc, G128, ln=bp + "norm2", bias=False, kind="qkv")
            ck, cvt, T, ldc_vt = self.ctx_kv[bp]
            a = rec.empty(M, Cc)
            rec.attention(q, ck, cvt, a, B, self.heads, d, HW, T, Cc, Cc, ldc_vt, Cc, HW * Cc, T * Cc, Cc * ldc_vt, HW * Cc, scale)
            self.attention_ip(bp, q, a, B, HW, Cc, d, scale)
            h = proj(a, bp + "attn2.to_out.0", Cc, Cc, G128, R=h, ldr=Cc, kind="attn_out")
        if opt("gw_ff1_g256") and self.g256_tile(M, 8 * Cc, Cc, dict(act=_lib.ACT_GEGLU)):
            ln = rec.layernorm(h, M, Cc, pw.f[bp + "norm3.weight"], pw.f[bp + "norm3.bias"], 1e-5)
            g = self.dense(ln, M, Cc, bp + "ff.net.0.proj", 8 * Cc, act=_lib.ACT_GEGLU, kind="ff")
        else:
            g = proj(h, bp + "ff.net.0.proj", 8 * Cc, Cc, G128, ln=bp + "norm3", act=_lib.ACT_GEGLU, kind="ff")
        if rec.lib.bc_gemm_wreg_eligible(M, Cc, 5 * Cc, 4 * Cc, G128):
            k = pw.ff2_proj_out(p)
            out = proj(g, k, Cc, 5 * Cc, G128, A2=h, C1=4 * Cc, lda=4 * Cc, lda2=Cc, R=x.t, ldr=Cc, kind="ff", rows_per_batch=HW, want_gn=True,
                       **self._r2(r2, x.H, x.W))
            return Act(out, Cc, x.H, x.W), None
        h = proj(g, bp + "ff.net.2", Cc, 4 * Cc, G128, R=h, ldr=Cc, kind="ff")
        out = proj(h, p + "proj_out", Cc, Cc, G128, R=x.t, ldr=Cc, kind="conv1x1", rows_per_batch=HW, want_gn=True, **self._r2(r2, x.H, x.W))
        return Act(out, Cc, x.H, x.W), None

    def transformer(self, p, x: Act, r2=None, zero=None):
        rec, pw, B = self.rec, self.pw, self.B
        Cc, HW = x.C, x.H * x.W
        M = B * HW
        if self.rowchain_ok(Cc, M, HW, p):
            return self.transformer_rowchain(p, x, r2, zero)
        if Cc % 320 == 0 and HW % 64 == 0 and self.gw_tile(M, Cc, Cc):
            return self.transformer_gw(p, x, r2)
        d = Cc // self.heads
        scale = d ** -0.5
        bp = p + "transformer_blocks.0."
        n = self.groupnorm(x, None, p + "norm", 1e-6, False)
        h = self.dense(n.t, M, Cc, p + "proj_in", Cc, kind="conv1x1")
        ln = rec.layernorm(h, M, Cc, pw.f[bp + "norm1.weight"], pw.f[bp + "norm1.bias"], 1e-5)
        ldvt = (HW + 63) // 64 * 64
        vt = rec.zeros(B, Cc, ldvt)
        qkv_kw = dict(C_t=vt, ldc_t=ldvt, n_t0=2 * Cc, rows_per_batch=HW)
        if self.g256_tile(M, 3 * Cc, Cc, qkv_kw):
            qk = rec.empty(M, 2 * Cc)
            rec.gemm(A=ln, W=pw.h[pw.qkv_weight(bp)], M=M, N=3 * Cc, K=Cc, out=qk, tile_cfg=_lib.TILE_G256, kind="qkv", **qkv_kw)
        else:
            qk = self.dense(ln, M, Cc, None, 2 * Cc, bias=False, wkey=bp + "attn1.to_qk.weight", kind="qkv")
            self.dense(ln, M, Cc, None, Cc, bias=False, wkey=bp + "attn1.to_v.weight", out=vt, out_mode=_lib.OUT_F16_T,
                       ldc=ldvt, rows_per_batch=HW, kind="qkv")
        a = rec.empty(M, Cc)
        self.self_attention(p, qk, vt, a, B, d, HW, Cc, ldvt, scale)
        h = self.dense(a, M, Cc, bp + "attn1.to_out.0", Cc, R=h, ldr=Cc, kind="attn_out")
        if pw.has_cross:
            ln = rec.layernorm(h, M, Cc, pw.f[bp + "norm2.weight"], pw.f[bp + "norm2.bias"], 1e-5)
            q = self.dense(ln, M, Cc, None, Cc, bias=False, wkey=bp + "attn2.to_q.weight", kind="qkv")
            ck, cvt, T, ldc_vt = self.ctx_kv[bp]
            a = rec.empty(M, Cc)
            rec.attention(q, ck, cvt, a, B, self.heads, d, HW, T, Cc, Cc, ldc_vt, Cc, HW * Cc, T * Cc, Cc * ldc_vt,
                          HW * Cc, scale)
            self.attention_ip(bp, q, a, B, HW, Cc, d, scale)
            h = self.dense(a, M, Cc, bp + "attn2.to_out.0", Cc, R=h, ldr=Cc, kind="attn_out")
        ln = rec.layernorm(h, M, Cc, pw.f[bp + "norm3.weight"], pw.f[bp + "norm3.bias"], 1e-5)
        g = self.dense(ln, M, Cc, bp + "ff.net.0.proj", 8 * Cc, act=_lib.ACT_GEGLU, kind="ff")
        r2kw = self._r2(r2, x.H, x.W)
        fused_kw = dict(A2=h, C1=4 * Cc, lda=4 * Cc, lda2=Cc, R=x.t, ldr=Cc, rows_per_batch=HW, want_gn=True, **r2kw)
        if self.g256_tile(M, Cc, 5 * Cc, fused_kw):
            k = pw.ff2_proj_out(p)
            out = rec.empty(M, Cc)
            rec.gemm(A=g, W=pw.h[k + ".weight"], M=M, N=Cc, K=5 * Cc, out=out, bias=pw.f[k + ".bias"], tile_cfg=_lib.TILE_G256, kind="ff", **fused_kw)
# ... 314 lines not shown
```

blobctrl_amd/launch.py:

```python
import ctypes as C
import json
import os
import struct
from typing import List, Optional

import torch

from . import _lib
from .options import opt
from ._lib import BcGemm


_TUNING_PATH = os.environ.get("BC_TUNING_FILE") or os.path.join(os.path.dirname(os.path.abspath(__file__)), "gemm_tuning.json")
_TUNING = None
_M64 = (1 << 64) - 1


def tuning_table():
    global _TUNING
    if _TUNING is None:
        _TUNING = {}
        if os.path.exists(_TUNING_PATH) and not os.environ.get("BC_NO_TUNING"):
            with open(_TUNING_PATH) as f:
                _TUNING = json.load(f).get("shapes", {})
# ... 398 lines not shown
        elif tile_cfg == _lib.TILE_G256:
            mode = "g256" + ("_qkv" if C_t is not None else "") + ("_2src" if A2 is not None else "")
        else:
            mode = "dense"
            if conv:
                ups = (conv.get("Hv", conv["Hin"]), conv.get("Wv", conv["Win"])) != (conv["Hin"], conv["Win"])
                mode = "ups" if ups else f"conv{conv.get('stride', 1)}"
            if tile_cfg == 0 and splitk is None and info.family == _lib.FAMILIES.index("gemm_fast"):
                hit = tuning_table().get(f"{mode}|{M}|{N}|{K}")
                if hit:
                    g.tile_cfg, g.splitk = int(hit[0]), int(hit[1])
        info = self.resolve(g, kind)
        g.tile_cfg = info.tile_cfg
        if not Cs:
            g.splitk = info.splitk
        sk = info.splitk
        if sk > 1:
            self.reserve_slab(info.slab_elems)
        part = None
        if want_gn and info.stat_rows:
            rpb = rows_per_batch if rows_per_batch > 0 else (conv["Hout"] * conv["Wout"] if conv else M)
            part = gn_tot_out if gn_tot_out is not None else self.new_tot(M // rpb, n_out)
            assert tuple(part.shape[:2]) == (M // rpb, n_out)
            g.gn_tot = part.data_ptr()
            self.tots[g.C] = part

        idx = self.lib.bc_plan_add_gemm(self.plan, self.seg.id, self.sid, C.byref(g))
        if idx < 0 or idx != len(self.seg.meta):
            _lib.check(1, "bc_plan_add_gemm")
        refs = (A, A2, W, out, bias, R, R2, rowvec, rowvec_idx, colscale, alpha_dev, alpha_idx, part, a_affine, ln_colsum, C_t, S, S2)
        self.keep.append(refs)
        for t in refs:
            self.register(t)
        variant = f"{_lib.FAMILIES[info.family]}_kernel<{_lib.TILE_NAMES[info.tile_cfg]},{mode}>" + ("+splitk_reduce" if sk > 1 else "")
        rp = info.kernel.decode()
        a_elems = (M // (conv["Hout"] * conv["Wout"])) * conv["Hin"] * conv["Win"] * conv["Cin"] if conv else M * K
        alg_bytes = 2 * (a_elems + N * K + M * n_out) + (2 * M * n_out if R is not None else 0) + 2 * (M + N) * Cs
        self._push(kind, 2 * M * N * (K + Cs), variant, (mode, M, N, K + Cs, sk), alg_bytes, rp)
        return out

    def _op(self, name, args, kind, **meta):
        self._add_op(_lib.op_code(name), _lib.op_signature(name), args, kind, **meta)

    def gn_sources(self, x1, C1, x2, C2, B, HW, G):
        srcs = []
        c2_ = C2 if x2 is not None else 0
        cpg = (C1 + c2_) // G
        for x, c, off in ((x1, C1, 0), (x2, c2_, C1)):
            if x is None:
                srcs.append(None)
                continue
            hit = self.tots.get(x.data_ptr())
            blocks_ok = c % 320 != 0 or id(hit) in self.tots_per_channel or (cpg % 10 == 0 and off % 10 == 0)
            if hit is not None and hit.shape[1] == c and blocks_ok:
                srcs.append(hit)
            else:
                tot = self.new_tot(B, c)
                self.keep.append((x, tot))
                self._op("bc_gn_stats", (x, c, B, HW, tot), "gn_stats", variant="gn_stats_kernel",
                         shape=("gn_stats", B, HW, c), bytes_=B * HW * c * 2)
                self.tots[x.data_ptr()] = tot
                self.tots_per_channel.add(id(tot))
                srcs.append(tot)
        return tuple(srcs)

    def groupnorm(self, x1, C1, x2, C2, B, HW, G, eps, gamma, beta, silu, out=None):
        c2 = C2 if x2 is not None else 0
        Cc = C1 + c2
        if out is None:
            out = self.empty(B, HW, Cc)
        n_before = self.seg.kinds.get("gn_stats", 0)
        t1, t2 = self.gn_sources(x1, C1, x2, c2, B, HW, G)
        own_stats = self.seg.kinds.get("gn_stats", 0) > n_before
        fused = not os.environ.get("BC_GN_UNFUSED") and Cc // G <= 96
        self.keep.append((x1, x2, t1, t2, gamma, beta, out))
        kind = "groupnorm" + ("" if own_stats else "_fused_stats")
        if fused:
            self._op("bc_gn_apply_fused", (t1, C1, t2, c2, x1, x2, B, HW, G, eps, gamma, beta, 1 if silu else 0, out), kind,
                     variant="gn_apply_fused_kernel", shape=("gn", B, HW, Cc), bytes_=2 * B * HW * Cc * 2)
        else:
            ab = self.empty(B, Cc, 2, dtype=torch.float32)
            self.keep.append(ab)
            self._op("bc_gn_finalize", (t1, C1, t2, c2, B, HW, G, eps, gamma, beta, ab), "gn_finalize",
                     variant="gn_finalize_kernel", shape=("gn_ab", B, HW, Cc))
            self._op("bc_gn_apply", (x1, C1, x2, c2, B, HW, ab, 1 if silu else 0, out), kind, variant="gn_apply_kernel",
                     shape=("gn", B, HW, Cc), bytes_=2 * B * HW * Cc * 2)
        return out

    def gn_affine(self, x1, C1, x2, C2, B, HW, G, eps, gamma, beta):
        c2 = C2 if x2 is not None else 0
        Cc = C1 + c2
        ab = self.empty(B, Cc, 2, dtype=torch.float32)
        t1, t2 = self.gn_sources(x1, C1, x2, c2, B, HW, G)
        self.keep.append((x1, x2, t1, t2, ab, gamma, beta))
        self._op("bc_gn_finalize", (t1, C1, t2, c2, B, HW, G, eps, gamma, beta, ab), "gn_finalize",
                 variant="gn_finalize_kernel", shape=("gn_ab", B, HW, Cc))
        return ab

    def layernorm(self, x, rows, Cc, gamma, beta, eps, out=None, ldx=None, ldy=None):
        if out is None:
            out = self.empty(rows, Cc)
        self.keep.append((x, gamma, beta, out))
        self._op("bc_layernorm", (x, rows, Cc, ldx or Cc, gamma, beta, eps, out, ldy or Cc), "layernorm", variant="layernorm_kernel",
                 shape=("ln", rows, Cc), bytes_=2 * rows * Cc * 2)
        return out

    def attention(self, Q, K, Vt, out, B, heads, d, Nq, Nkv, ldq, ldk, ldvt, ldo, qbs, kbs, vbs, obs, scale,
                  q_off=0, k_off=0, causal=False):
        self.keep.append((Q, K, Vt, out))
        self._op("bc_attention_causal" if causal else "bc_attention",
                 (Q.data_ptr() + q_off * 2, K.data_ptr() + k_off * 2, Vt, out, B, heads, d, Nq, Nkv, ldq, ldk, ldvt, ldo, qbs, kbs, vbs,
                  obs, scale), "attention", flops=4 * B * heads * Nq * Nkv * d, variant=f"attn_fwd_kernel<{d}>",
                 shape=(B, heads, d, Nq, Nkv), bytes_=2 * B * heads * d * (2 * Nq + 2 * Nkv))
        return out

    def attention_identity(self, Vt, out, B, b0, HW, Cc, ldvt, ldo):
        self.keep.append((Vt, out))
        for t in (Vt, out):
            self.register(t)
        self._op("bc_attention_identity", (Vt, out, B, b0, HW, Cc, ldvt, ldo), "attention_identity", variant="attention_identity_kernel",
                 shape=("attention_identity", B - b0, HW, Cc), bytes_=2 * 2 * (B - b0) * HW * Cc)
        return out

    def attention_ip(self, Q, K, V, out, B, rows_per_batch, heads, d, T, ldq, ldkv, ldo, scale, w, q_off=0):
        Cc = heads * d
        self.keep.append((Q, K, V, out, w))
        for t in (Q, K, V, out, w):
            self.register(t)
        tiles = T % 16 == 0 and _lib.load().bc_attention_ip_path(d, T, rows_per_batch, heads) == _lib.ATTENTION_IP_TILES
        variant = f"attention_ip_tiles_kernel<{d},{T // 16}>" if tiles else f"attention_ip_kernel<{d}>"
        self._op("bc_attention_ip", (Q.data_ptr() + q_off * 2, K, V, out, B, rows_per_batch, heads, d, T, ldq, ldkv, ldo, scale, w),
                 "attention_ip", flops=4 * B * rows_per_batch * T * Cc, variant=variant,
                 shape=("attention_ip", B, heads, d, rows_per_batch, T), bytes_=2 * (3 * B * rows_per_batch * Cc + 2 * B * T * Cc))
        return out

    def attention_ip_masked(self, Q, K, V, out, B, rows_per_batch, heads, d, images, tokens_per_image, ldq, ldkv, ldo, scale, w, mask, ldm, q_off=0):
        Cc, T = heads * d, images * tokens_per_image
        self.keep.append((Q, K, V, out, w, mask))
        for t in (Q, K, V, out, w, mask):
            self.register(t)
        tiles = _lib.load().bc_attention_ip_masked_path(d, images, tokens_per_image, rows_per_batch, heads) == _lib.ATTENTION_IP_TILES
        variant = f"attention_ip_masked_tiles_kernel<{d},{T // 16}>" if tiles else f"attention_ip_masked_kernel<{d}>"
        self._op("bc_attention_ip_masked", (Q.data_ptr() + q_off * 2, K, V, out, B, rows_per_batch, heads, d, images, tokens_per_image, ldq, ldkv,
                                            ldo, scale, w, mask, ldm),
                 "attention_ip_masked", flops=4 * B * rows_per_batch * T * Cc, variant=variant,
                 shape=("attention_ip_masked", B, heads, d, rows_per_batch, images, tokens_per_image),
                 bytes_=2 * (3 * B * rows_per_batch * Cc + 2 * B * T * Cc + images * rows_per_batch))
        return out

    def rowchain(self, kind, Cc, M, rows_per_batch, x, wstream, vec, out0, out1=None, out2=None, ldvt=0, affine=None, gn_in=None, res=None, res2=None,
                 r2=None, r2_xmin=0, r2_bmod=1, out_w=0, gn_tot=None, ln_eps=1e-5, alpha=1.0, alpha_dev=None, alpha_idx=None,
                 alpha_bstride=0, part=None, nsplit=1):
        mult = {_lib.CHAIN_IN: 4, _lib.CHAIN_MID: 2, _lib.CHAIN_OUT: 14 + (1 if out1 is not None else 0), _lib.CHAIN_OUT_FF: 13,
                _lib.CHAIN_OUT_TAIL: 1 + (1 if out1 is not None else 0), _lib.CHAIN_OUT_FFP: 14 + (1 if out1 is not None else 0)}[kind]
        g_tot, g_gamma, g_beta, g_groups, g_eps = gn_in if gn_in is not None else (None, None, None, 0, 0.0)
        refs = (x, wstream, vec, out0, out1, out2, affine, res, res2, r2, gn_tot, alpha_dev, alpha_idx, part, g_tot, g_gamma, g_beta)
        self.keep.append(refs)
        for t in refs:
            self.register(t)
        name = {_lib.CHAIN_IN: "in", _lib.CHAIN_MID: "mid", _lib.CHAIN_OUT: "out", _lib.CHAIN_OUT_FF: f"out_ff/{nsplit}", _lib.CHAIN_OUT_TAIL: "out_tail",
                _lib.CHAIN_OUT_FFP: f"out_ffp/{nsplit}"}[kind]
        zk = (_lib.CHAIN_OUT, _lib.CHAIN_OUT_TAIL, _lib.CHAIN_OUT_FFP)
        self._op("bc_rowchain", (kind, Cc, M, rows_per_batch, x, affine, g_tot, g_gamma, g_beta, g_groups, g_eps, res, res2, r2, r2_xmin, r2_bmod, out_w, wstream, vec, out0, out1, out2,
                                 ldvt, gn_tot, ln_eps, alpha, alpha_dev, alpha_idx, alpha_bstride, part, nsplit), "rowchain",
                 flops=2 * M * Cc * Cc * mult,
                 variant=f"rowchain_kernel<{name}{',zero' if kind in zk and out1 is not None else ''}>",
                 shape=("rowchain_" + name, M, Cc, mult * Cc), bytes_=2 * (mult * Cc * Cc + 2 * M * Cc),
                 rocprof=f"rowchain_kernel<{Cc}, {kind}, {'true' if kind in zk and out1 is not None else 'false'}>")
        return out0

    def rowchain_sum(self, Cc, M, rows_per_batch, part, nsplit, out0, gn_tot=None, out1=None):
        refs = (part, out0, gn_tot, out1)
        self.keep.append(refs)
        for t in refs:
            self.register(t)
        nout = 2 if out1 is not None else 1
        self._op("bc_rowchain_sum", (Cc, M, rows_per_batch, part, nsplit, out0, gn_tot, out1), "rowchain_sum", variant="rowchain_sum_kernel",
                 shape=("rowchain_sum", M, Cc, nsplit), bytes_=2 * nout * (nsplit + 1) * M * Cc, rocprof=f"rowchain_sum_kernel<{Cc}>")
        return out0

    def rowchain_kv_stream(self, ck, cvt, B, T, Cc, ldvt):
        frags = self.lib.bc_rowchain_kv_frags(Cc)
        if frags < 0:
            _lib.check(1, "bc_rowchain_kv_frags")
        out = self.empty(B * (Cc // 80) * frags * 64 * 8)
        self.keep.append((ck, cvt, out))
        self._op("bc_rowchain_pack_kv", (ck, Cc, cvt, ldvt, B, T, Cc, out), "pack_kv", variant="rowchain_pack_kv_kernel",
                 shape=("pack_kv", B, T, Cc), bytes_=2 * (2 * B * T * Cc) + out.numel() * 2, rocprof=f"rowchain_pack_kv_kernel<{Cc}>")
        return out

    def ctx_fold(self, ck, cvt, B, T, Cc, ldvt, heads, scale, wq, bq, wo):
        N = 128 * heads
        s_qk, s_vo = self.lib.bc_gemm_wreg_stream_elems(N, Cc), self.lib.bc_gemm_wreg_stream_elems(Cc, 80 * heads)
        wqk, vwo = self.zeros(B, s_qk), self.zeros(B, s_vo)
        cs, qb = self.zeros(B, N, dtype=torch.float32), self.zeros(B, N, dtype=torch.float32)
        refs = (ck, cvt, wq, bq, wo, wqk, cs, qb, vwo)
        self.keep.append(refs)
        for t in refs:
            self.register(t)
        self._op("bc_ctx_fold", (ck, Cc, cvt, ldvt, B, T, Cc, heads, scale, wq, bq, wo, wqk, cs, qb, vwo), "ctx_fold", variant="ctx_fold_kernel",
                 flops=2 * 2 * B * 80 * heads * Cc * (Cc // heads), shape=("ctx_fold", B, T, Cc), bytes_=2 * (2 * Cc * Cc + B * (N + 80 * heads) * Cc),
                 rocprof="ctx_fold_qk_kernel")
        return wqk, cs, qb, vwo

    def rowchain_midx(self, Cc, M, rows_per_batch, x, wstream, vec, kvstream, n_ctx, heads, scale, out0, out1, res, ln_eps=1e-5):
        assert heads * (Cc // heads) == Cc and heads == 8, "CHAIN_MIDX is laid out for 8 heads"
        refs = (x, wstream, vec, kvstream, out0, out1, res)
        self.keep.append(refs)
        for t in refs:
            self.register(t)
        B = M // rows_per_batch
        self._op("bc_rowchain_midx", (Cc, M, rows_per_batch, x, res, wstream, vec, kvstream, n_ctx, scale, out0, out1, ln_eps), "rowchain",
                 flops=2 * M * Cc * Cc * 2 + 4 * M * n_ctx * Cc, variant="rowchain_kernel<midx>",
                 shape=("rowchain_midx", M, Cc, 2 * Cc), bytes_=2 * (2 * Cc * Cc + 3 * M * Cc + 2 * B * n_ctx * Cc),
                 rocprof=f"rowchain_kernel<{Cc}, {_lib.CHAIN_MIDX}, false>")
        return out1

    def call(self, name, *args, kind=None, keep=()):
        self.keep.append(keep)
        for t in keep if isinstance(keep, (tuple, list)) else (keep,):
            self.register(t)
        self._op(name, args, kind or name)
```

blobctrl_amd/weights.py:

```python
from collections import OrderedDict
from typing import Dict, Optional

import torch


def pad8(n: int) -> int:
    return (n + 7) // 8 * 8


def merge_lora(sd: Dict[str, torch.Tensor], lora: Dict[str, torch.Tensor], alphas: Optional[Dict[str, float]] = None,
               adapter_scale: float = 1.0) -> Dict[str, torch.Tensor]:
    out = OrderedDict((k, v.clone()) for k, v in sd.items())
    for key in list(lora.keys()):
        if not key.endswith(".lora_A.weight"):
            continue
        mod = key[: -len(".lora_A.weight")]
        a = lora[key].float()
        b = lora[mod + ".lora_B.weight"].float()
        r = b.shape[1]
        alpha = float(alphas.get(mod, r)) if alphas else float(r)
        w = out[mod + ".weight"]
        delta = (b.flatten(1) @ a.flatten(1)).reshape(w.shape)
        out[mod + ".weight"] = w + (adapter_scale * alpha / r) * delta
    return out
# ... 241 lines not shown
                continue
            if ".time_emb_proj.weight" in k:
                p = k[: -len("time_emb_proj.weight")]
                temb_w.append(v)
                temb_b.append(sd[p + "time_emb_proj.bias"])
                self.temb_slices[p] = (off, v.shape[0])
                off += v.shape[0]
            elif ".ff.net.0.proj.weight" in k:
                w, b = interleave_geglu(v, sd[k[:-6] + "bias"])
                self.h[k] = w.half().to(device)
                self.f[k[:-6] + "bias"] = b.to(device)
            elif k.endswith("attn1.to_q.weight"):
                p = k[: -len("to_q.weight")]
                self.h[p + "to_qk.weight"] = torch.cat([v, sd[p + "to_k.weight"]], 0).half().to(device)
            elif k.endswith("attn1.to_k.weight"):
                continue
            elif v.ndim == 4 and v.shape[-1] == 3:
                self.h[k] = pack_conv3x3(v).half().to(device)
            else:
                self.h[k] = pack_matrix(v).half().to(device)
        self.temb_total = off
        w_in = sd["conv_in.weight"]
        co = w_in.shape[0]

        def k128(w8ch):
            out = torch.zeros(co, 128)
            out[:, :72] = w8ch.reshape(co, 72)
            return out
        if w_in.shape[1] <= 8:
            base = torch.zeros(co, 3, 3, 8)
            base[..., : w_in.shape[1]] = w_in.permute(0, 2, 3, 1)
            self.h["conv_in.weight_k128"] = k128(base).half().to(device)
        if w_in.shape[1] > 8:
            base = torch.zeros(co, 3, 3, 8)
            base[..., :5] = w_in[:, :5].permute(0, 2, 3, 1)
            self.h["conv_in.weight8"] = k128(base).half().to(device)
            fm = torch.zeros(co, 16, w_in.shape[1] - 5)
            fm[:, :9] = w_in[:, 5:].permute(0, 2, 3, 1).reshape(co, 9, -1)
            self.h["conv_in.featmat"] = pack_matrix(fm.reshape(co * 16, -1)).half().to(device)
        self.h["temb_all.weight"] = torch.cat(temb_w, 0).half().to(device)
        self.f["temb_all.bias"] = torch.cat(temb_b, 0).to(device)
        self._to_arenas()

    @staticmethod
    def _layout(tensors, align_elems):
        layout, off = [], 0
        for k, t in tensors.items():
            layout.append((k, tuple(t.shape), off))
            off += (t.numel() + align_elems - 1) // align_elems * align_elems
        return layout, off

    def _to_arenas(self):
        self.h_layout, hn = self._layout(self.h, 128)
        self.f_layout, fn = self._layout(self.f, 64)
        self.h_arena = torch.zeros(hn, dtype=torch.float16, device=self.device)
        self.f_arena = torch.zeros(fn, dtype=torch.float32, device=self.device)
        self._view(copy_from=(self.h, self.f))

    def _view(self, copy_from=None):
        h, f = {}, {}
        for (k, shape, off) in self.h_layout:
            n = 1
            for d in shape:
                n *= d
            h[k] = self.h_arena[off:off + n].view(shape)
            if copy_from is not None:
                h[k].copy_(copy_from[0][k])
        for (k, shape, off) in self.f_layout:
            n = 1
            for d in shape:
                n *= d
            f[k] = self.f_arena[off:off + n].view(shape)
            if copy_from is not None:
                f[k].copy_(copy_from[1][k])
        self.h, self.f = h, f

    def meta(self):
        return dict(h_layout=self.h_layout, f_layout=self.f_layout, temb_slices=self.temb_slices,
                    temb_total=self.temb_total, has_cross=self.has_cross, boc=self.boc,
                    h_elems=self.h_arena.numel(), f_elems=self.f_arena.numel())

    @classmethod
    def from_meta(cls, meta, device):
        self = cls.__new__(cls)
        self.device = device
        self.h_layout, self.f_layout = meta["h_layout"], meta["f_layout"]
        self.temb_slices, self.temb_total = meta["temb_slices"], meta["temb_total"]
        self.has_cross, self.boc = meta["has_cross"], meta["boc"]
        self.h_arena = torch.zeros(meta["h_elems"], dtype=torch.float16, device=device)
        self.f_arena = torch.zeros(meta["f_elems"], dtype=torch.float32, device=device)
        self._view()
        return self

    def derived_nbytes(self):
        n = sum(t.numel() * t.element_size() for k, t in self.h.items() if k.endswith("_wreg"))
        for cache in (self.__dict__.get("_gw", {}), self.__dict__.get("_rowchain", {}), self.__dict__.get("_ctx_fold", {})):
            for v in cache.values():
                n += sum(t.numel() * t.element_size() for t in v if torch.is_tensor(t))
        return n

    def nbytes(self):
        return self.h_arena.numel() * 2 + self.f_arena.numel() * 4 + self.derived_nbytes()


RC_HC, RC_RPAD = 128, 20
RC_CHANNELS = (320, 640)


def _frag_stream(w: torch.Tensor, row_starts, k0: int = 0, k1: int = None) -> torch.Tensor:
    k1 = w.shape[1] if k1 is None else k1
    rs = torch.as_tensor(row_starts, device=w.device)
    nw, nt = rs.shape
    rows = rs[:, :, None] + torch.arange(16, device=w.device)
    x = w[rows.reshape(-1), k0:k1].reshape(nw, nt, 16, (k1 - k0) // 32, 4, 8)
    return x.permute(0, 3, 1, 4, 2, 5).reshape(nw, -1, 64, 8).contiguous()


def pack_rowchain_kv(k: torch.Tensor, vt: torch.Tensor, T: int, pad_frags: int = 20) -> torch.Tensor:
    B, _, C = k.shape
    D = C // 8
    hpw, qks, vtiles = 80 // D, (2 if D == 40 else 3), (3 if D == 40 else 5)
    fr_head = 5 * qks + 3 * vtiles
    nw = C // 80
    out = torch.zeros(B, nw, hpw * fr_head + pad_frags, 64, 8, dtype=torch.float16, device=k.device)
    kp = torch.zeros(B, 80, C + 64, dtype=torch.float16, device=k.device)
    kp[:, :T, :C] = k[:, :T]
    vp = torch.zeros(B, C, 96, dtype=torch.float16, device=k.device)
    vp[:, :, :T] = vt[:, :, :T]
    lane = torch.arange(64, device=k.device)
    m, q = lane % 16, lane // 16
    j = torch.arange(8, device=k.device)
    for w in range(nw):
        for hh in range(hpw):
            c_h = 80 * w + D * hh
            s0 = c_h // 32
            f0 = hh * fr_head
            for ks in range(qks):
                for t in range(5):
                    ch = 32 * (s0 + ks) + 8 * q[:, None] + j[None, :]
                    val = kp[:, (16 * t + m)[:, None].expand(64, 8), ch]
                    inside = (ch >= c_h) & (ch < c_h + D)
                    out[:, w, f0 + ks * 5 + t] = torch.where(inside[None], val, torch.zeros_like(val))
            tlo = 2 if (D == 40 and hh == 1) else 0
            for ks in range(3):
                for tv in range(vtiles):
                    chv = 80 * w + 16 * (tlo + tv) + m
                    key = 32 * ks + 8 * q[:, None] + j[None, :]
                    val = vp[:, chv[:, None].expand(64, 8), key]
                    inside = ((chv >= c_h) & (chv < c_h + D))[:, None].expand(64, 8)
                    out[:, w, f0 + 5 * qks + ks * vtiles + tv] = torch.where(inside[None], val, torch.zeros_like(val))
    return out


def pack_rowchain(pw: "PackedTrunk", p: str, kind: int, zero_name: Optional[str] = None, nsplit: int = 1):
    h, f = pw.h, pw.f
    bp = p + "transformer_blocks.0."
    C = h[p + "proj_in.weight"].shape[0]
    assert C in RC_CHANNELS, C
    nw = C // 80
    nC = [[80 * w + 16 * t for t in range(5)] for w in range(nw)]
    segs, vec = [], []
    if kind == 0:
        qk = h[bp + "attn1.to_qk.weight"]
        segs = [_frag_stream(h[p + "proj_in.weight"], nC), _frag_stream(qk[:C], nC), _frag_stream(qk[C:], nC),
                _frag_stream(h[bp + "attn1.to_v.weight"], nC)]
        vec = [f[p + "proj_in.bias"], f[bp + "norm1.weight"], f[bp + "norm1.bias"]]
    elif kind == 1:
        segs = [_frag_stream(h[bp + "attn1.to_out.0.weight"], nC), _frag_stream(h[bp + "attn2.to_q.weight"], nC)]
        vec = [f[bp + "attn1.to_out.0.bias"], f[bp + "norm2.weight"], f[bp + "norm2.bias"]]
    else:
        att = "attn2" if pw.has_cross else "attn1"
        w1i, b1i = h[bp + "ff.net.0.proj.weight"], f[bp + "ff.net.0.proj.bias"]
        hid = 4 * C
        w1 = w1i.reshape(hid // 32, 2, 32, C)
        b1 = b1i.reshape(hid // 32, 2, 32)
        wv, wg = w1[:, 0].reshape(hid, C), w1[:, 1].reshape(hid, C)
        bv, bg = b1[:, 0].reshape(hid), b1[:, 1].reshape(hid)
        w1o = torch.cat([wv, wg], 0)
        w2 = h[bp + "ff.net.2.weight"]
        seg_to_out = _frag_stream(h[bp + att + ".to_out.0.weight"], nC)
        ffb, chunks = [], []
        hpw = RC_HC // nw
        for c in range(hid // RC_HC):
            cs = []
            for tp in range(hpw // 16):
                cs.append(_frag_stream(w1o, [[RC_HC * c + hpw * w + 16 * tp, hid + RC_HC * c + hpw * w + 16 * tp] for w in range(nw)]))
            cs.append(_frag_stream(w2, nC, RC_HC * c, RC_HC * (c + 1)))
            chunks.append(cs)
            for w in range(nw):
                for tp in range(hpw // 16):
                    j0 = RC_HC * c + hpw * w + 16 * tp
                    ffb += [bv[j0:j0 + 16], bg[j0:j0 + 16]]
        seg_proj_out = _frag_stream(h[p + "proj_out.weight"], nC)
        if kind == 2:
            segs = [seg_to_out] + [x for cs in chunks for x in cs] + [seg_proj_out]
        elif kind == 4:
            segs = [seg_proj_out]
        vec = [f[bp + att + ".to_out.0.bias"], f[bp + "norm3.weight"], f[bp + "norm3.bias"], torch.cat(ffb), f[bp + "ff.net.2.bias"],
               f[p + "proj_out.bias"]]
        seg_zero = None
        if zero_name is not None:
            seg_zero = _frag_stream(h[zero_name + ".weight"], nC)
            if kind not in (3, 6):
                segs.append(seg_zero)
            vec.append(f[zero_name + ".bias"])
        if kind in (3, 6):
            nchunks = len(chunks)
            assert nchunks % nsplit == 0, (nchunks, nsplit)
            pad = torch.zeros(nw, RC_RPAD, 64, 8, dtype=torch.float16, device=seg_to_out.device)
            per = nchunks // nsplit
            tail = ([seg_proj_out] + ([seg_zero] if seg_zero is not None else [])) if kind == 6 else []
            slices = [torch.cat([seg_to_out] + [x for cs in chunks[z * per:(z + 1) * per] for x in cs] + tail + [pad], 1) for z in range(nsplit)]
            return torch.stack(slices).contiguous(), torch.cat([v.reshape(-1).float() for v in vec]).contiguous()
    pad = torch.zeros(nw, RC_RPAD, 64, 8, dtype=torch.float16, device=segs[0].device)
    return torch.cat(segs + [pad], 1).contiguous(), torch.cat([v.reshape(-1).float() for v in vec]).contiguous()


IP_NUM_TOKENS = 4


def ip_attn2_prefixes(keys):
    end = "attn2.to_k.weight"
    rank = {"down_blocks": 0, "up_blocks": 1, "mid_block": 2}

    def order(bp):
        parts = bp.split(".")
        nums = [int(x) for x in parts if x.isdigit()]
        return (rank[parts[0]], nums)
    return sorted((k[: -len(end)] for k in keys if k.endswith(end)), key=order)


IP_PLUS_DEPTH, IP_PLUS_DIM_HEAD = 4, 64

_PLUS_LAYER_KEYS = {
    "ln0_w": ("0.norm1.weight", "ln0.weight"), "ln0_b": ("0.norm1.bias", "ln0.bias"),
    "ln1_w": ("0.norm2.weight", "ln1.weight"), "ln1_b": ("0.norm2.bias", "ln1.bias"),
    "to_q": ("0.to_q.weight", "attn.to_q.weight"), "to_kv": ("0.to_kv.weight", None),
    "to_k": (None, "attn.to_k.weight"), "to_v": (None, "attn.to_v.weight"), "to_out": ("0.to_out.weight", "attn.to_out.0.weight"),
    "ff_ln_w": ("1.0.weight", "ff.0.weight"), "ff_ln_b": ("1.0.bias", "ff.0.bias"),
    "ff1": ("1.1.weight", "ff.1.net.0.proj.weight"), "ff2": ("1.3.weight", "ff.1.net.2.weight"),
}
_PLUS_TOP_KEYS = ("latents", "proj_in.weight", "proj_in.bias", "proj_out.weight", "proj_out.bias", "norm_out.weight", "norm_out.bias")


def ip_plus_layers(image_proj):
    if any(k not in image_proj for k in _PLUS_TOP_KEYS) or any(k.startswith(f"layers.{IP_PLUS_DEPTH}.") for k in image_proj):
        return None
    layers = []
    for i in range(IP_PLUS_DEPTH):
        which = 1 if f"layers.{i}.attn.to_q.weight" in image_proj else 0
        layer = {}
        for name, spell in _PLUS_LAYER_KEYS.items():
            if spell[which] is None:
                continue
            key = f"layers.{i}.{spell[which]}"
            if key not in image_proj:
                return None
            layer[name] = image_proj[key]
        if "to_kv" in layer:
            layer["to_k"], layer["to_v"] = layer.pop("to_kv").chunk(2, dim=0)
        layers.append(layer)
    return layers


def ip_adapter_layout(image_proj) -> str:
    if "proj.weight" in image_proj:
        return "base"
    if "latents" in image_proj and "perceiver_resampler.proj_in.weight" not in image_proj and "proj.3.weight" not in image_proj and \
            "norm.weight" not in image_proj and ip_plus_layers(image_proj) is not None:
        return "plus"
    if "proj.3.weight" in image_proj:
        what = "IP-Adapter Full Face (IPAdapterFullImageProjection)"
    elif "perceiver_resampler.proj_in.weight" in image_proj:
        what = "IP-Adapter FaceID Plus (IPAdapterFaceIDPlusImageProjection)"
    elif "norm.weight" in image_proj:
        what = "IP-Adapter FaceID (IPAdapterFaceIDImageProjection)"
    elif "latents" in image_proj:
        what = "IP-Adapter Plus (IPAdapterPlusImageProjection, a Resampler) with an incomplete projection"
    else:
        raise ValueError("not an IP-Adapter image projection: no proj.weight, proj.3.weight, perceiver_resampler, norm.weight or latents")
    raise NotImplementedError(f"{what} is not supported: only the base IP-Adapter (ImageProjection: proj.weight + norm) and a complete "
                              "IP-Adapter Plus projection are")


def ip_adapter_tokens(ad) -> int:
    return int(ad["latents"].shape[0]) if ad.get("layout") == "plus" else IP_NUM_TOKENS


def ip_adapter_embed_dim(ad) -> int:
    return int(ad["proj_in_w"].shape[1]) if ad.get("layout") == "plus" else int(ad["proj_w"].shape[1])


def convert_ip_adapter(sd, prefixes, ctx_dim):
    layout = ip_adapter_layout(sd["image_proj"])
    ip, proj = sd["ip_adapter"], sd["image_proj"]
    if any("_lora." in k for k in ip):
        raise NotImplementedError("IP-Adapter FaceID LoRA weights (to_k_lora / to_q_lora ...) are not supported")
    if layout == "base" and proj["proj.weight"].shape[0] != IP_NUM_TOKENS * ctx_dim:
        raise ValueError(f"image_proj.proj.weight has {proj['proj.weight'].shape[0]} rows; {IP_NUM_TOKENS} tokens of this UNet's "
                         f"cross_attention_dim {ctx_dim} need {IP_NUM_TOKENS * ctx_dim}")
    if layout == "plus" and proj["proj_out.weight"].shape[0] != ctx_dim:
        raise ValueError(f"image_proj.proj_out.weight has {proj['proj_out.weight'].shape[0]} rows; this UNet's cross_attention_dim is {ctx_dim}")
    want = {f"{1 + 2 * i}.to_{n}_ip.weight" for i in range(len(prefixes)) for n in "kv"}
    if set(ip) != want:
        raise ValueError(f"ip_adapter keys do not match this UNet's {len(prefixes)} attn2 processors: missing {sorted(want - set(ip))[:4]}, "
                         f"unexpected {sorted(set(ip) - want)[:4]}")
    kv = OrderedDict((bp, (ip[f"{1 + 2 * i}.to_k_ip.weight"].float(), ip[f"{1 + 2 * i}.to_v_ip.weight"].float())) for i, bp in enumerate(prefixes))
    if layout == "base":
        return dict(proj_w=proj["proj.weight"].float(), proj_b=proj["proj.bias"].float(), norm_w=proj["norm.weight"].float(),
                    norm_b=proj["norm.bias"].float(), kv=kv)
    hidden = proj["latents"].shape[2]
    layers = []
    for src in ip_plus_layers(proj):
        inner = src["to_q"].shape[0]
        if inner % IP_PLUS_DIM_HEAD or src["to_k"].shape != (inner, hidden) or src["to_out"].shape != (hidden, inner):
            raise ValueError(f"a Resampler layer with to_q {tuple(src['to_q'].shape)}, to_k {tuple(src['to_k'].shape)}, to_out "
                             f"{tuple(src['to_out'].shape)}: heads of {IP_PLUS_DIM_HEAD} over {hidden} hidden channels are expected")
        layer = {k: src[k].float() for k in ("ln0_w", "ln0_b", "ln1_w", "ln1_b", "to_v", "to_out", "ff_ln_w", "ff_ln_b", "ff1", "ff2")}
        layer["qk"] = torch.cat([src["to_q"].float(), src["to_k"].float()], 0)
        layers.append(layer)
    return dict(layout="plus", latents=proj["latents"].float().reshape(-1, hidden), proj_in_w=proj["proj_in.weight"].float(),
                proj_in_b=proj["proj_in.bias"].float(), layers=layers, proj_out_w=proj["proj_out.weight"].float(),
                proj_out_b=proj["proj_out.bias"].float(), norm_w=proj["norm_out.weight"].float(), norm_b=proj["norm_out.bias"].float(),
                heads=layers[0]["qk"].shape[0] // 2 // IP_PLUS_DIM_HEAD, kv=kv)


def ip_adapter_on_device(host, device):
    h16, f32 = torch.float16, torch.float32
    mat, vec = (lambda t: t.to(device, h16).contiguous()), (lambda t: t.to(device, f32).contiguous())
    out = dict(kv=OrderedDict((bp, (mat(wk), mat(wv))) for bp, (wk, wv) in host["kv"].items()),
               scales=torch.ones(len(host["kv"]), dtype=f32, device=device), norm_w=vec(host["norm_w"]), norm_b=vec(host["norm_b"]))
    if host.get("layout") == "plus":
        out.update(layout="plus", heads=host["heads"], latents=mat(host["latents"]), proj_in_w=mat(host["proj_in_w"]),
                   proj_in_b=vec(host["proj_in_b"]), proj_out_w=mat(host["proj_out_w"]), proj_out_b=vec(host["proj_out_b"]),
                   layers=[{k: (vec(v) if v.ndim == 1 else mat(v)) for k, v in layer.items()} for layer in host["layers"]])
    else:
        out.update(proj_w=mat(host["proj_w"]), proj_b=vec(host["proj_b"]))
    return out
```

include/blobctrl_hip.h:

```cpp
#ifndef BLOBCTRL_HIP_H
#define BLOBCTRL_HIP_H

#include <stdint.h>

#ifdef __cplusplus
extern "C" {
#endif

typedef uint16_t bc_half;
typedef void*    bc_stream;

const char* bc_last_error(void);
int bc_version(void);
int bc_device_info(int* out4);

enum { BC_A_DENSE = 0, BC_A_CONV3X3 = 1 };
enum { BC_ACT_NONE = 0, BC_ACT_GELU = 1, BC_ACT_GEGLU = 2, BC_ACT_SILU = 3, BC_ACT_QUICK_GELU = 4  };
enum { BC_OUT_F16 = 0, BC_OUT_F16_T = 1, BC_OUT_F32 = 2 };

typedef struct BcGemm {
    const bc_half* A;
    const bc_half* A2;
    int a_mode;
    int M, N, K;
// ... 10 lines not shown
    const float*   bias;
    const bc_half* rowvec;
    int ld_rowvec;
    int rows_per_batch;
    const int* rowvec_idx;
    int rowvec_step;
    int act;
    const float*   colscale;
    float alpha;
    const float*   alpha_dev;
    const int*     alpha_idx;
    int alpha_bstride;
    const bc_half* R;
    int ldr;
    const bc_half* R2;
    int ldr2, r2_xmin, r2_bmod, out_w;
    int out_mode;
    void* C;
    int ldc;
    int splitk;
    float* slab;
    unsigned long long* gn_tot;
    int tile_cfg;
    const float* a_affine;
    int a_act;
    const unsigned long long* a_tot1;
    const unsigned long long* a_tot2;
    const float* a_gamma; const float* a_beta;
    int a_groups; float a_eps;
    const float* ln_colsum; float ln_eps;
    void* C_t; int ldc_t, n_t0;
    long long w_bstride; int vec_bstride;
    int sm_group, sm_valid, sm_keep;
    const bc_half* S; const bc_half* S2;
    int lds, lds2, S1, Cs;
} BcGemm;

int bc_gemm(const BcGemm* p, bc_stream stream);
int bc_sizeof_gemm(void);
enum { BC_TILE_AUTO = 0, BC_TILE_256x128 = 1, BC_TILE_128x128_S3 = 2, BC_TILE_128x128_S2 = 3, BC_TILE_256x64_S2 = 4,
       BC_TILE_256x64_S3 = 5, BC_TILE_128x64 = 6, BC_TILE_64x64 = 7, BC_TILE_COUNT = 8,
       BC_TILE_HALO = 8,
       BC_TILE_WREG = 9,
       BC_TILE_GW64x128 = 10, BC_TILE_GW64x256 = 11, BC_TILE_GW64x320 = 12,
       BC_TILE_G256 = 13 };
int bc_gemm_wreg_pack(const bc_half* w, int ldw, int N, int K, int tile_cfg, bc_half* out, bc_stream stream);
long long bc_gemm_wreg_stream_elems(int N, int K);
int bc_gemm_wreg_eligible(int M, int N, int K, int C1, int tile_cfg);
int bc_gemm256_eligible(int M, int N, int K, int C1, int out_mode, int rows_per_batch, int want_gn);
int bc_conv_wreg_pack(const bc_half* w, int N, int Cin, bc_half* out, bc_stream stream);
int bc_conv_wreg_pack_sc(const bc_half* w, int N, int Cin, const bc_half* wsc, int Cs, bc_half* out, bc_stream stream);
int bc_conv_wreg_pack_host(const bc_half* w, int N, int Cin, const bc_half* wsc, int Cs, bc_half* out);
int bc_conv_wreg_sc_eligible(int Cin, int N, int H, int W, int Cs, int S1, int reserved);
int bc_conv_halo_eligible(int Cin, int C1, int N, int Hin, int Win, int Hout, int Wout, int stride);
int bc_conv_halo_max_chunks(void);
int bc_gemm_plan(int M, int N, int K, int fast, int* tile_cfg, int* splitk, int* bm, int* bn);
enum { BC_FAMILY_GENERIC = 0 , BC_FAMILY_FAST = 1 , BC_FAMILY_HALO = 2 ,
       BC_FAMILY_CONV_WREG = 3 , BC_FAMILY_GEMM_WREG = 4 , BC_FAMILY_G256 = 5  };
typedef struct BcGemmInfo {
    int family;
    int tile_cfg, bm, bn;
    int splitk;
    int n_out;
    long long slab_elems;
    int stat_rows;
    int gn_finalize_fits;
    char kernel[64];
} BcGemmInfo;
int bc_gemm_resolve(const BcGemm* in, BcGemmInfo* out);

enum { BC_GN_TOT_WORDS = 6 };
int bc_gn_stats(const bc_half* x, int C, int B, int HW, unsigned long long* tot, bc_stream stream);
int bc_gn_finalize(const unsigned long long* tot1, int C1, const unsigned long long* tot2, int C2, int B, int HW, int G,
                   float eps, const float* gamma, const float* beta, float* ab, bc_stream stream);
int bc_gn_apply(const bc_half* x1, int C1, const bc_half* x2, int C2, int B, int HW,
                const float* ab, int silu, bc_half* y, bc_stream stream);
int bc_gn_apply_fused(const unsigned long long* tot1, int C1, const unsigned long long* tot2, int C2,
                      const bc_half* x1, const bc_half* x2, int B, int HW, int G, float eps, const float* gamma,
                      const float* beta, int silu, bc_half* y, bc_stream stream);
int bc_memset_zero(void* ptr, long long bytes, bc_stream stream);
int bc_dup_halves(void* p0, long long bytes0, void* p1, long long bytes1, void* p2, long long bytes2, void* p3, long long bytes3,
                  void* p4, long long bytes4, void* p5, long long bytes5, bc_stream stream);

int bc_freeu(const bc_half* hidden, int C_h, const bc_half* skip, int C_s, int B, int HW, const float* params, int stage,
             const float* basis, bc_half* hidden_out, bc_half* skip_out, unsigned long long* tot_h, unsigned long long* tot_s,
             bc_stream stream);

int bc_softmax_rows(bc_half* x, int rows, int cols, int ld, bc_stream stream);

int bc_embed_tokens(const long long* ids, const bc_half* tok_emb, const float* pos_emb, int B, int T, int D, int vocab,
                    bc_half* out, bc_stream stream);

int bc_gaussian_sample(const bc_half* moments, const float* noise, int B, int Cz, int HW, float scale, float* out,
                       bc_stream stream);

int bc_layernorm(const bc_half* x, int rows, int C, int ldx, const float* gamma, const float* beta, float eps,
                 bc_half* y, int ldy, bc_stream stream);

int bc_attention(const bc_half* Q, const bc_half* K, const bc_half* Vt, bc_half* O,
                 int B, int heads, int d, int Nq, int Nkv,
                 int ldq, int ldk, int ldvt, int ldo,
                 long long q_bstride, long long k_bstride, long long vt_bstride, long long o_bstride,
                 float scale, bc_stream stream);
int bc_attention_causal(const bc_half* Q, const bc_half* K, const bc_half* Vt, bc_half* O,
                        int B, int heads, int d, int Nq, int Nkv,
                        int ldq, int ldk, int ldvt, int ldo,
                        long long q_bstride, long long k_bstride, long long vt_bstride, long long o_bstride,
                        float scale, bc_stream stream);
int bc_attention_build(int d, int B, int heads, int Nq, int Nkv, int causal);

int bc_splat_scores(const double* params_host, int n, int h, int w, double* out, bc_stream stream);

int bc_splat_maps(const double* params_host, int n, int h, int w, double* raw, double* composed, bc_stream stream);
int bc_alpha_composite(const double* raw, long long npix, int K, double* out, bc_stream stream);
int bc_splat_from_scores(const void* S, const void* F, int N, int M, int C, int Hin, int Win, long long s_n, long long s_m,
                         long long s_y, long long s_x, int Hout, int Wout, int is_f32, void* out, bc_stream stream);
int bc_resize_bilinear(const void* in, long long planes, int Hin, int Win, int Hout, int Wout, int is_f32, void* out,
                       bc_stream stream);
int bc_pack_rgb8(const double* img, int H, int W, unsigned char* out, bc_stream stream);

int bc_assemble_input(const float* latents, int Blat, const float* img_lat, const float* score, const float* feat,
                      int Bimg, int F, int Bout, int h, int w, int Cpad, int dup_score, bc_half* X, bc_stream stream);
int bc_assemble_input_im2col(const float* latents, int Blat, const float* img_lat, const float* score, int Bimg, int Bout,
                             int h, int w, int dup_score, bc_half* X, bc_stream stream);
int bc_assemble_input_scaled(const float* latents, int Blat, const float* img_lat, const float* score, const float* feat,
                             int Bimg, int F, int Bout, int h, int w, int Cpad, int dup_score, const float* coef, const int* step_idx,
                             int nsteps, bc_half* X, bc_stream stream);
int bc_assemble_input_im2col_scaled(const float* latents, int Blat, const float* img_lat, const float* score, int Bimg, int Bout,
                                    int h, int w, int dup_score, const float* coef, const int* step_idx, int nsteps, bc_half* X,
                                    bc_stream stream);

int bc_timestep_embedding(const float* t_table, const int* t_idx, float t_value, int rows, int dim, bc_half* out,
                          bc_stream stream);
int bc_timestep_embedding_table(const float* t_table, int nsteps, int rows_per_step, int dim, bc_half* out, bc_stream stream);
int bc_timestep_embedding_cond(const float* t_table, const int* t_idx, float t_value, int rows, int dim, const float* cond,
                               bc_half* out, bc_stream stream);
int bc_timestep_embedding_table_cond(const float* t_table, int nsteps, int rows_per_step, int dim, const float* cond, bc_half* out,
                                     bc_stream stream);

int bc_silu(const bc_half* x, bc_half* y, long long n, bc_stream stream);

int bc_cfg_scheduler_step(const float* eps, float* latents, const float* coef, int* step_idx, float* hist,
                          float guidance_scale, int B, int h, int w, float* eps_out, int advance, bc_stream stream);

int bc_cfg_scheduler_step_noise(const float* eps, float* latents, const float* coef, int* step_idx, float* hist,
                                float guidance_scale, int B, int h, int w, const float* noise, int nsteps, float* eps_out,
                                int advance, bc_stream stream);

int bc_cfg_scheduler_step3(const float* eps, float* latents, const float* coef, int* step_idx, float* hist,
                           float guidance_scale, int B, int h, int w, int nsteps, float* eps_out, int advance, bc_stream stream);
int bc_scheduler_step_single(const float* eps, float* latents, const float* coef, int* step_idx, float* hist, int B, int h, int w,
                             const float* noise, int nsteps, int third, float* eps_out, int advance, bc_stream stream);

enum { BC_CHAIN_IN = 0, BC_CHAIN_MID = 1, BC_CHAIN_OUT = 2, BC_CHAIN_OUT_FF = 3, BC_CHAIN_OUT_TAIL = 4, BC_CHAIN_MIDX = 5, BC_CHAIN_OUT_FFP = 6 };
int bc_rowchain_supported(int channels, int M, int rows_per_batch);
long long bc_rowchain_stream_frags(int channels, int kind, int blobnet, int nsplit);
int bc_rowchain(int kind, int channels, int M, int rows_per_batch, const bc_half* x, const float* affine,
                const unsigned long long* gn_in, const float* gn_gamma, const float* gn_beta, int gn_groups, float gn_eps, const bc_half* res,
                const bc_half* res2, const bc_half* r2, int r2_xmin, int r2_bmod, int out_w, const bc_half* wstream,
                const float* vec, bc_half* out0, bc_half* out1, bc_half* out2, int ldvt, unsigned long long* gn_tot, float ln_eps,
                float alpha, const float* alpha_dev, const int* alpha_idx, int alpha_bstride, float* part, int nsplit, bc_stream stream);
int bc_rowchain_sum(int channels, int M, int rows_per_batch, const bc_half* part, int nsplit, bc_half* out0, unsigned long long* gn_tot,
                    bc_half* out1, bc_stream stream);
long long bc_rowchain_kv_frags(int channels);
int bc_rowchain_pack_kv(const bc_half* k, int ldk, const bc_half* vt, int ldvt, int B, int T, int channels, bc_half* out, bc_stream stream);

int bc_ctx_fold(const bc_half* k, int ldk, const bc_half* vt, int ldvt, int B, int T, int channels, int heads, float scale,
                const bc_half* wq, const float* bq, const bc_half* wo, bc_half* wqk, float* qk_colsum, float* qk_bias, bc_half* vwo,
                bc_stream stream);
int bc_rowchain_midx(int channels, int M, int rows_per_batch, const bc_half* x, const bc_half* res, const bc_half* wstream, const float* vec,
                     const bc_half* kvstream, int n_ctx, float attn_scale, bc_half* out0, bc_half* out1, float ln_eps, bc_stream stream);

int bc_nchw_to_nhwc_f16(const void* src, int src_is_f32, int B, int C, int HW, int Cpad, bc_half* dst, bc_stream stream);
int bc_nhwc_to_nchw(const bc_half* src, int B, int C, int HW, int ldsrc, void* dst, int dst_is_f32, bc_stream stream);
int bc_add_cls_pos(const bc_half* patches, const float* cls, const float* pos, int B, int T, int D, bc_half* out,
                   bc_stream stream);
int bc_patchify(const float* pixels, int B, int H, int W, int patch, int Kpad, bc_half* out, bc_stream stream);

int bc_graph_begin(bc_stream stream);
int bc_graph_end(bc_stream stream, void** graph_exec_out);
int bc_graph_launch(void* graph_exec, bc_stream stream);
int bc_graph_destroy(void* graph_exec);

int bc_event_create_sync(void** ev);
int bc_stream_wait_event(bc_stream stream, void* ev);

int bc_event_create(void** ev);
int bc_event_record(void* ev, bc_stream stream);
int bc_event_elapsed_ms(void* start, void* stop, float* ms);
int bc_event_destroy(void* ev);

typedef struct BcPlan BcPlan;
enum { BC_OP_GEMM = 0, BC_OP_GN_STATS = 1, BC_OP_GN_FINALIZE = 2, BC_OP_GN_APPLY_FUSED = 3, BC_OP_GN_APPLY = 4, BC_OP_LAYERNORM = 5,
       BC_OP_ATTENTION = 6, BC_OP_ATTENTION_CAUSAL = 7, BC_OP_ASSEMBLE_INPUT = 8, BC_OP_TIMESTEP_EMBEDDING = 9,
       BC_OP_TIMESTEP_EMBEDDING_TABLE = 10, BC_OP_CFG_SCHEDULER_STEP = 11, BC_OP_EMBED_TOKENS = 12, BC_OP_SOFTMAX_ROWS = 13,
       BC_OP_PATCHIFY = 14, BC_OP_ADD_CLS_POS = 15, BC_OP_SILU = 16, BC_OP_NCHW_TO_NHWC_F16 = 17, BC_OP_NHWC_TO_NCHW = 18,
       BC_OP_GAUSSIAN_SAMPLE = 19, BC_OP_SIGNAL = 20 , BC_OP_WAIT = 21 , BC_OP_ROWCHAIN = 22, BC_OP_ASSEMBLE_IM2COL = 23,
       BC_OP_MEMSET_ZERO = 24, BC_OP_ROWCHAIN_MIDX = 25, BC_OP_ROWCHAIN_PACK_KV = 26, BC_OP_ROWCHAIN_SUM = 27, BC_OP_CTX_FOLD = 28, BC_OP_DUP_HALVES = 29,
       BC_OP_CFG_SCHEDULER_STEP_NOISE = 30, BC_OP_CFG_SCHEDULER_STEP3 = 31, BC_OP_ASSEMBLE_INPUT_SCALED = 32,
       BC_OP_ASSEMBLE_IM2COL_SCALED = 33, BC_OP_SCHEDULER_STEP_SINGLE = 34, BC_OP_TIMESTEP_EMBEDDING_TABLE_COND = 35,
       BC_OP_TIMESTEP_EMBEDDING_COND = 36, BC_OP_FREEU = 37,
       BC_OP_SCHEDULER_STEP_REQUESTS = 38, BC_OP_ASSEMBLE_INPUT_REQUESTS = 39,
       BC_OP_ASSEMBLE_IM2COL_REQUESTS = 40, BC_OP_TIMESTEP_EMBEDDING_ROWS = 41,
       BC_OP_ATTENTION_RELPOS = 42, BC_OP_WINDOW_PARTITION = 43, BC_OP_WINDOW_UNPARTITION = 44, BC_OP_ADD_POS = 45, BC_OP_ADD_ROWS = 46,
       BC_OP_ACT_ROWS = 47, BC_OP_BILINEAR_RESIZE_F32 = 48, BC_OP_SAM_TOKENS = 49, BC_OP_SAM_MASKS = 50,
       BC_OP_SAM_TOKENS_BATCH = 51, BC_OP_MASK_STATS = 52, BC_OP_COUNT = 53 };
typedef struct BcPlanBuffer {
    const char* name;
    const void* address;
    long long   bytes;
    const void* host_data;
} BcPlanBuffer;

int bc_plan_create(BcPlan** out);
int bc_plan_destroy(BcPlan* plan);
int bc_plan_segment(BcPlan* plan, const char* name);
int bc_plan_find_segment(BcPlan* plan, const char* name);
int bc_plan_new_event(BcPlan* plan);
int bc_plan_add_gemm(BcPlan* plan, int seg, int stream_id, const BcGemm* g);
int bc_plan_add_op(BcPlan* plan, int seg, int stream_id, int op, const uint64_t* args, int nargs);
int bc_plan_set_slab(BcPlan* plan, int stream_id, float* slab);
int bc_plan_enable(BcPlan* plan, int seg, int index, int enabled);
int bc_plan_num_launches(BcPlan* plan, int seg);
int bc_step(BcPlan* plan, int seg, const bc_stream* streams, int nstreams);
int bc_plan_capture(BcPlan* plan, int seg, const bc_stream* streams, int nstreams);
int bc_plan_release(BcPlan* plan, int seg);
int bc_plan_capture_loop(BcPlan* plan, const int* seg_sequence, int n, const bc_stream* streams, int nstreams, void** graph_exec_out);
int bc_plan_run_timed(BcPlan* plan, int seg, bc_stream stream, float* ms_out );
int bc_plan_run_timed_kernels(BcPlan* plan, int seg, bc_stream stream, float* ms_main, float* ms_reduce);
int bc_plan_run_marked(BcPlan* plan, int seg, const bc_stream* streams, int nstreams, const int* marks, int nmarks, float* ms_out);
int bc_plan_save(BcPlan* plan, const char* path, const BcPlanBuffer* buffers, int nbuffers);
int bc_plan_load(const char* path, BcPlan** out);
int bc_plan_buffer(BcPlan* plan, const char* name, void** ptr, long long* bytes);

#ifdef __cplusplus
}
#endif
#endif
```

Measured before the change: 2.445.

## Fold proj_out into FF down-projection weights for split rowchain output

Adds a new rowchain output kind that precomputes proj_out·W2 and the matching folded bias at weight-pack time. Each split slice applies its share of proj_out to the attention output h2 via a ring-streamed GEMM segment, so the separate per-row proj_out GEMM after the feed-forward is dropped. This removes one full C×C GEMM pass and its LDS round-trip from the serial tail of each slice. In exchange it adds a small GEMM segment per slice, keeps an fp16 product of two weight matrices (possible precision change), and adds more complex LDS placement that needs nsplit >= 2.

```diff
diff --git a/blobctrl_amd/_lib.py b/blobctrl_amd/_lib.py
--- a/blobctrl_amd/_lib.py
+++ b/blobctrl_amd/_lib.py
@@ -306,7 +306,7 @@
 PAG_OPS = {"bc_attention_identity": 60, "bc_pag_scheduler_step": 61}
 _OP_TABLES_PAG = (PAG_OPS,)
 OP_SIGNAL, OP_WAIT = 20, 21
-CHAIN_IN, CHAIN_MID, CHAIN_OUT, CHAIN_OUT_FF, CHAIN_OUT_TAIL, CHAIN_MIDX, CHAIN_OUT_FFP = 0, 1, 2, 3, 4, 5, 6
+CHAIN_IN, CHAIN_MID, CHAIN_OUT, CHAIN_OUT_FF, CHAIN_OUT_TAIL, CHAIN_MIDX, CHAIN_OUT_FFP, CHAIN_OUT_FFPF = 0, 1, 2, 3, 4, 5, 6, 7
 GN_TOT_WORDS = 6
 _KIND = {C.c_void_p: "p", C.c_int: "i", C.c_float: "f", C.c_longlong: "l", C.c_char_p: "p"}
 
diff --git a/blobctrl_amd/csrc/rowchain.hip b/blobctrl_amd/csrc/rowchain.hip
--- a/blobctrl_amd/csrc/rowchain.hip
+++ b/blobctrl_amd/csrc/rowchain.hip
@@ -7,6 +7,7 @@
 constexpr int RC_BM = 64;
 constexpr int RC_NT = 5;
 constexpr int RC_HC = 128;
+constexpr int RC_T_FFPF = 6, RC_T_FFP = 7;
 constexpr int RC_RPAD = 20;
 
 template <int C>
@@ -24,6 +25,7 @@
     static constexpr int NPASS = RC_BM / ROWS_PASS;
     static constexpr int NKC = C / 64;
     static constexpr int G = RC_NT * KS;
+    static constexpr int R_FF = C == 320 ? 15 : 10;
 };
 
 struct RowChainArgs {
@@ -126,6 +128,35 @@
     __builtin_amdgcn_sched_barrier(0);
 }
 
+constexpr int ffp_seg_frags(int nks, int ring) { return (RC_NT * nks + ring - 1) / ring * ring; }
+
+template <int NT, int POS, int RC_R>
+__device__ __forceinline__ void gemm_seg_rings(f32x4v (&acc)[NT][4], WRing<RC_R>& r, const char* xb, int nks) {
+    static_assert(RC_R % NT == 0, "a ring must hold whole k-steps");
+    constexpr int PER = RC_R / NT;
+    for (int s0 = 0; s0 < nks; s0 += PER) {
+#pragma unroll
+        for (int j = 0; j < PER; ++j) {
+            if (s0 + j < nks) {
+                h16x8 xq[4];
+#pragma unroll
+                for (int mt = 0; mt < 4; ++mt) xq[mt] = *reinterpret_cast<const h16x8*>(xb + (s0 + j) * 4096 + mt * 1024);
+#pragma unroll
+                for (int t = 0; t < NT; ++t) {
+                    const h16x8 w = as_h8(r.f[(POS + j * NT + t) % RC_R]);
+#pragma unroll
+                    for (int mt = 0; mt < 4; ++mt) acc[t][mt] = __builtin_amdgcn_mfma_f32_16x16x32_f16(w, xq[mt], acc[t][mt], 0, 0, 0);
+                }
+            }
+            __builtin_amdgcn_sched_barrier(0);
+#pragma unroll
+            for (int t = 0; t < NT; ++t) r.f[(POS + j * NT + t) % RC_R] = r.p[t * 64];
+            r.p += NT * 64;
+            __builtin_amdgcn_sched_barrier(0);
+        }
+    }
+}
+
 template <int NT, int KS, int POS, int RC_R, int JUMP>
 __device__ __forceinline__ void gemm_seg_jump(f32x4v (&acc)[NT][4], WRing<RC_R>& r, const uint4* p2, const char* xb) {
     h16x8 xq[2][4];
@@ -335,6 +366,20 @@
         for (int mt = 0; mt < 4; ++mt) {
             const float v[4] = {acc[t][mt][0], acc[t][mt][1], acc[t][mt][2], acc[t][mt][3]};
             *reinterpret_cast<h16x4*>(X + x_off(c0 >> 5, 16 * mt + m, (c0 & 31) >> 3) + ((c0 >> 2) & 1) * 8) = pack4(v);
+        }
+    }
+}
+
+__device__ __forceinline__ void acc_ksteps_to_X(const f32x4v (&acc)[RC_NT][4], char* img, int k0, int nks, int wave, int m, int q) {
+#pragma unroll
+    for (int t = 0; t < RC_NT; ++t) {
+        const int rel = ((80 * wave + 16 * t) >> 5) - k0;
+        if (rel < 0 || rel >= nks) continue;
+        const int c0 = 80 * wave + 16 * t + 4 * q;
+#pragma unroll
+        for (int mt = 0; mt < 4; ++mt) {
+            const float v[4] = {acc[t][mt][0], acc[t][mt][1], acc[t][mt][2], acc[t][mt][3]};
+            *reinterpret_cast<h16x4*>(img + x_off(rel, 16 * mt + m, (c0 & 31) >> 3) + ((c0 >> 2) & 1) * 8) = pack4(v);
         }
     }
 }
@@ -430,7 +475,8 @@
     const int lane = tid & 63;
     const int wave = __builtin_amdgcn_readfirstlane(tid >> 6);
     const int m = lane & 15, q = lane >> 4;
-    constexpr bool FFP = KIND == BC_CHAIN_OUT_FFP;
+    constexpr bool FOLD = KIND == RC_T_FFPF;
+    constexpr bool FFP = KIND == RC_T_FFP || FOLD;
     constexpr bool FF = KIND == BC_CHAIN_OUT_FF || FFP, TAIL = KIND == BC_CHAIN_OUT_TAIL;
     const int wg = bc_xcd_remap(blockIdx.x, gridDim.x);
     const int nrb = a.M / RC_BM;
@@ -511,8 +557,8 @@
     }
     constexpr bool FFLOOP = KIND == BC_CHAIN_OUT || FF;
     constexpr bool MIDX = KIND == BC_CHAIN_MIDX;
-    constexpr int RC_R = RC_C == 320 ? (FFLOOP ? 15 : (KIND == BC_CHAIN_IN ? 13 : (MIDX ? 12 : 16)))
-                                     : (FFLOOP ? 10 : (KIND == BC_CHAIN_IN ? 12 : (MIDX ? 8 : 12)));
+    constexpr int RC_R = FFLOOP ? CF::R_FF : RC_C == 320 ? (KIND == BC_CHAIN_IN ? 13 : (MIDX ? 12 : 16))
+                                                         : (KIND == BC_CHAIN_IN ? 12 : (MIDX ? 8 : 12));
     static_assert(RC_R <= RC_RPAD, "stream padding");
     WRing<RC_R> ring;
     ring.p = a.wstream + ((size_t)z * CF::NW + wave) * a.wave_frags * 64 + lane;
@@ -666,19 +712,25 @@
     }
 
     if (!TAIL) {
+    constexpr int POS_FF = (RC_NT * RC_KS) % RC_R;
     layernorm_to_X<RC_C>(acc, vec + RC_C, a.ln_eps, X, wave, m, q);
+    const int nks = FOLD ? RC_KS / a.nsplit : 0;
+    if constexpr (FOLD) {
+        static_assert(RC_KS == RC_NCH && 16384 + RC_KS / 2 * 4096 <= CF::S_BYTES, "the share of h2 of one slice of two must fit behind the first hidden chunk");
+        acc_ksteps_to_X(acc, S + 16384, z * nks, nks, wave, m, q);
+    }
     lds_barrier();
     stamp(3);
-    if (FF && z != 0) zero_acc(acc);
+    if (FOLD || (FF && z != 0)) zero_acc(acc);
+    if constexpr (FOLD) gemm_seg_rings<RC_NT, POS_FF>(acc, ring, S + 16384 + xfo, nks);
     const int c_lo = FF ? z * (RC_NCH / a.nsplit) : 0, c_hi = FF ? c_lo + RC_NCH / a.nsplit : RC_NCH;
     {
         const float* b1 = vec + 3 * RC_C;
-        constexpr int POS_FF = (RC_NT * RC_KS) % RC_R;
         constexpr int TP = CF::TP, HPW = CF::HW_;
         static_assert(!FFLOOP || (TP * 2 * RC_KS + RC_NT * (RC_HC / 32)) % RC_R == 0,
                       "a feed-forward chunk must consume a whole number of rings");
         for (int c = c_lo; c < c_hi; ++c) {
-            char* P = S + (c & 1) * 16384;
+            char* P = S + ((FOLD ? c - c_lo : c) & 1) * 16384;
             const float* bb = b1 + (c * CF::NW + wave) * (2 * HPW) + 4 * q;
             float4 bvg[2 * TP];
 #pragma unroll
@@ -744,16 +796,23 @@
 #define xfo xfo_
 #define cm cm_
     const bool first = !FFP || z == 0;
-    if (first) epi_bias_res<RC_C, false>(acc, vec + 3 * RC_C + 8 * RC_C, S, wave, m, q);
-    lds_barrier();
-    acc_to_X(acc, X, wave, m, q);
-    if (first) rows_to_S<RC_C>(a.res2 + (size_t)m0 * RC_C, S, cm);
-    lds_barrier();
-    zero_acc(acc);
     constexpr int POS_PO = TAIL ? 0 : (RC_NT * RC_KS) % RC_R;
-    stamp(5);
-    gemm_seg<RC_NT, RC_KS, POS_PO, true>(acc, ring, X + xfo);
-    stamp(6);
+    constexpr int POS_ZERO = (POS_PO + (FOLD ? 0 : RC_NT * RC_KS)) % RC_R;
+    if constexpr (!FOLD) {
+        if (first) epi_bias_res<RC_C, false>(acc, vec + 3 * RC_C + 8 * RC_C, S, wave, m, q);
+        lds_barrier();
+        acc_to_X(acc, X, wave, m, q);
+        if (first) rows_to_S<RC_C>(a.res2 + (size_t)m0 * RC_C, S, cm);
+        lds_barrier();
+        zero_acc(acc);
+        stamp(5);
+        gemm_seg<RC_NT, RC_KS, POS_PO, true>(acc, ring, X + xfo);
+        stamp(6);
+    } else if (first) {
+        lds_barrier();
+        rows_to_S<RC_C>(a.res2 + (size_t)m0 * RC_C, S, cm);
+        lds_barrier();
+    }
     const float* bpo = vec + 3 * RC_C + 8 * RC_C + RC_C;
     if (first) epi_bias_res<RC_C, true>(acc, bpo, S, wave, m, q);
     if (a.r2 && first) {
@@ -776,7 +835,7 @@
         S_to_X<RC_C>(S, X, cm);
         lds_barrier();
         zero_acc(acc);
-        gemm_seg<RC_NT, RC_KS, (POS_PO + RC_NT * RC_KS) % RC_R, true>(acc, ring, X + xfo);
+        gemm_seg<RC_NT, RC_KS, POS_ZERO, true>(acc, ring, X + xfo);
         if (first) epi_bias_res<RC_C, false>(acc, bpo + RC_C, S, wave, m, q);
         float alpha = a.alpha;
         if (a.alpha_dev) alpha *= a.alpha_dev[(a.alpha_idx ? *a.alpha_idx : 0) * (a.alpha_bstride > 0 ? a.alpha_bstride : 1) + (a.alpha_bstride > 0 ? b : 0)];
@@ -833,7 +892,7 @@
     RcStampReport report{stream, nwg, a.stamps, KIND};
     static std::atomic<unsigned long long> lds_set{0};
     BC_CHECK_HIP(bc_set_max_lds(lds_set, reinterpret_cast<const void*>(&rowchain_kernel<RC_C, KIND, BLOB>), CF::LDS));
-    hipLaunchKernelGGL((rowchain_kernel<RC_C, KIND, BLOB>), dim3(a.M / RC_BM * (KIND == BC_CHAIN_OUT_FF || KIND == BC_CHAIN_OUT_FFP ? a.nsplit : 1)), dim3(CF::NTH), CF::LDS, stream, a);
+    hipLaunchKernelGGL((rowchain_kernel<RC_C, KIND, BLOB>), dim3(a.M / RC_BM * (KIND == BC_CHAIN_OUT_FF || KIND == RC_T_FFP || KIND == RC_T_FFPF ? a.nsplit : 1)), dim3(CF::NTH), CF::LDS, stream, a);
     BC_CHECK_LAUNCH();
     return 0;
 }
@@ -910,6 +969,8 @@
     else if (kind == BC_CHAIN_OUT) n = 2 * g + CF::NCH * per_chunk + (blobnet ? g : 0);
     else if (kind == BC_CHAIN_OUT_FF && nsplit > 0 && CF::NCH % nsplit == 0) n = g + CF::NCH / nsplit * per_chunk;
     else if (kind == BC_CHAIN_OUT_FFP && nsplit > 0 && CF::NCH % nsplit == 0) n = 2 * g + CF::NCH / nsplit * per_chunk + (blobnet ? g : 0);
+    else if (kind == BC_CHAIN_OUT_FFPF && nsplit > 0 && CF::NCH % nsplit == 0)
+        n = g + ffp_seg_frags(CF::KS / nsplit, CF::R_FF) + CF::NCH / nsplit * per_chunk + (blobnet ? g : 0);
     else if (kind == BC_CHAIN_OUT_TAIL) n = g + (blobnet ? g : 0);
     else return -1;
     return n + RC_RPAD;
@@ -922,7 +983,8 @@
         case BC_CHAIN_MID: return launch_chain<RC_C, BC_CHAIN_MID, false>(a, s);
         case BC_CHAIN_OUT_FF: return launch_chain<RC_C, BC_CHAIN_OUT_FF, false>(a, s);
         case BC_CHAIN_OUT_TAIL: return blob ? launch_chain<RC_C, BC_CHAIN_OUT_TAIL, true>(a, s) : launch_chain<RC_C, BC_CHAIN_OUT_TAIL, false>(a, s);
-        case BC_CHAIN_OUT_FFP: return blob ? launch_chain<RC_C, BC_CHAIN_OUT_FFP, true>(a, s) : launch_chain<RC_C, BC_CHAIN_OUT_FFP, false>(a, s);
+        case BC_CHAIN_OUT_FFP: return blob ? launch_chain<RC_C, RC_T_FFP, true>(a, s) : launch_chain<RC_C, RC_T_FFP, false>(a, s);
+        case BC_CHAIN_OUT_FFPF: return blob ? launch_chain<RC_C, RC_T_FFPF, true>(a, s) : launch_chain<RC_C, RC_T_FFPF, false>(a, s);
         default: return blob ? launch_chain<RC_C, BC_CHAIN_OUT, true>(a, s) : launch_chain<RC_C, BC_CHAIN_OUT, false>(a, s);
     }
 }
@@ -947,11 +1009,12 @@
                            bc_stream stream) {
     BC_CHECK_ARG(bc_rowchain_supported(channels, M, rows_per_batch), "bc_rowchain: needs 320 or 640 channels, M %% rows_per_batch == 0 and "
                  "rows_per_batch %% %d == 0 (channels=%d M=%d rows_per_batch=%d)", RC_BM, channels, M, rows_per_batch);
-    BC_CHECK_ARG((kind >= BC_CHAIN_IN && kind <= BC_CHAIN_OUT_TAIL) || kind == BC_CHAIN_OUT_FFP, "bc_rowchain: unknown kind %d", kind);
-    BC_CHECK_ARG(wstream && vec && (x || kind == BC_CHAIN_OUT_TAIL) && (out0 || kind == BC_CHAIN_OUT_FF || kind == BC_CHAIN_OUT_FFP),
+    const bool ffp = kind == BC_CHAIN_OUT_FFP || kind == BC_CHAIN_OUT_FFPF;
+    BC_CHECK_ARG((kind >= BC_CHAIN_IN && kind <= BC_CHAIN_OUT_TAIL) || ffp, "bc_rowchain: unknown kind %d", kind);
+    BC_CHECK_ARG(wstream && vec && (x || kind == BC_CHAIN_OUT_TAIL) && (out0 || kind == BC_CHAIN_OUT_FF || ffp),
                  "bc_rowchain: null pointer");
-    const bool blob = (kind == BC_CHAIN_OUT || kind == BC_CHAIN_OUT_TAIL || kind == BC_CHAIN_OUT_FFP) && out1 != nullptr;
-    if (kind == BC_CHAIN_OUT_FF || kind == BC_CHAIN_OUT_TAIL || kind == BC_CHAIN_OUT_FFP)
+    const bool blob = (kind == BC_CHAIN_OUT || kind == BC_CHAIN_OUT_TAIL || ffp) && out1 != nullptr;
+    if (kind == BC_CHAIN_OUT_FF || kind == BC_CHAIN_OUT_TAIL || ffp)
         BC_CHECK_ARG(part && nsplit >= 1 && (4 * channels / 128) % nsplit == 0, "bc_rowchain(OUT_FF / OUT_TAIL): needs the partial-sum buffer and nsplit "
                      "dividing the %d hidden chunks (nsplit=%d)", 4 * channels / 128, nsplit);
     RowChainArgs a;
@@ -976,8 +1039,10 @@
         BC_CHECK_ARG(out1 && out2 && ldvt >= rows_per_batch && ldvt % 8 == 0, "bc_rowchain(IN): needs out1 (q|k), out2 (V^T) and ldvt >= rows_per_batch, ldvt %% 8 == 0");
     if (kind == BC_CHAIN_MID) BC_CHECK_ARG(res && out1, "bc_rowchain(MID): needs res and out1");
     if (kind == BC_CHAIN_OUT_FF) BC_CHECK_ARG(res, "bc_rowchain(OUT_FF): needs res");
-    if (kind == BC_CHAIN_OUT_FFP) {
+    if (ffp) {
         BC_CHECK_ARG(res && res2 && !gn_tot, "bc_rowchain(OUT_FFP): needs res and res2; the statistics totals belong to bc_rowchain_sum");
+        BC_CHECK_ARG(kind == BC_CHAIN_OUT_FFP || nsplit >= 2, "bc_rowchain(OUT_FFPF): needs nsplit >= 2 (a slice's share of h2 must fit beside a hidden "
+                     "chunk; one workgroup per row block is BC_CHAIN_OUT)");
         BC_CHECK_ARG(!r2 || (out_w > 0 && rows_per_batch % out_w == 0), "bc_rowchain(OUT_FFP): r2 needs out_w dividing rows_per_batch");
     }
     if (kind == BC_CHAIN_OUT || kind == BC_CHAIN_OUT_TAIL) {
diff --git a/blobctrl_amd/engine.py b/blobctrl_amd/engine.py
--- a/blobctrl_amd/engine.py
+++ b/blobctrl_amd/engine.py
@@ -363,9 +363,9 @@
         nsplit = self.rowchain_ff_split(Cc, M)
         if nsplit > 1 and self.rowchain_ffp():
             pp = rec.empty((2 if zero is not None else 1) * nsplit, M, Cc)
-            w, v = packed(_lib.CHAIN_OUT_FFP, zname, nsplit)
+            w, v = packed(_lib.CHAIN_OUT_FFPF, zname, nsplit)
             kw2 = {k: v_ for k, v_ in kw.items() if k != "out1"}
-            rec.rowchain(_lib.CHAIN_OUT_FFP, Cc, M, HW, a, w, v, None, out1=res_out, res=h, res2=x.t, part=pp, nsplit=nsplit, **kw2)
+            rec.rowchain(_lib.CHAIN_OUT_FFPF, Cc, M, HW, a, w, v, None, out1=res_out, res=h, res2=x.t, part=pp, nsplit=nsplit, **kw2)
             rec.rowchain_sum(Cc, M, HW, pp, nsplit, out, gn_tot=part, out1=res_out)
         elif nsplit > 1:
             ffp = rec.empty(nsplit, M, Cc, dtype=torch.float32)
diff --git a/blobctrl_amd/launch.py b/blobctrl_amd/launch.py
--- a/blobctrl_amd/launch.py
+++ b/blobctrl_amd/launch.py
@@ -574,21 +574,23 @@
                  r2=None, r2_xmin=0, r2_bmod=1, out_w=0, gn_tot=None, ln_eps=1e-5, alpha=1.0, alpha_dev=None, alpha_idx=None,
                  alpha_bstride=0, part=None, nsplit=1):
         mult = {_lib.CHAIN_IN: 4, _lib.CHAIN_MID: 2, _lib.CHAIN_OUT: 14 + (1 if out1 is not None else 0), _lib.CHAIN_OUT_FF: 13,
-                _lib.CHAIN_OUT_TAIL: 1 + (1 if out1 is not None else 0), _lib.CHAIN_OUT_FFP: 14 + (1 if out1 is not None else 0)}[kind]
+                _lib.CHAIN_OUT_TAIL: 1 + (1 if out1 is not None else 0), _lib.CHAIN_OUT_FFP: 14 + (1 if out1 is not None else 0),
+                _lib.CHAIN_OUT_FFPF: 14 + (1 if out1 is not None else 0)}[kind]
         g_tot, g_gamma, g_beta, g_groups, g_eps = gn_in if gn_in is not None else (None, None, None, 0, 0.0)
         refs = (x, wstream, vec, out0, out1, out2, affine, res, res2, r2, gn_tot, alpha_dev, alpha_idx, part, g_tot, g_gamma, g_beta)
         self.keep.append(refs)
         for t in refs:
             self.register(t)
         name = {_lib.CHAIN_IN: "in", _lib.CHAIN_MID: "mid", _lib.CHAIN_OUT: "out", _lib.CHAIN_OUT_FF: f"out_ff/{nsplit}", _lib.CHAIN_OUT_TAIL: "out_tail",
-                _lib.CHAIN_OUT_FFP: f"out_ffp/{nsplit}"}[kind]
-        zk = (_lib.CHAIN_OUT, _lib.CHAIN_OUT_TAIL, _lib.CHAIN_OUT_FFP)
+                _lib.CHAIN_OUT_FFP: f"out_ffp/{nsplit}", _lib.CHAIN_OUT_FFPF: f"out_ffp/{nsplit}"}[kind]
+        zk = (_lib.CHAIN_OUT, _lib.CHAIN_OUT_TAIL, _lib.CHAIN_OUT_FFP, _lib.CHAIN_OUT_FFPF)
+        tag = {_lib.CHAIN_OUT_FFP: 7, _lib.CHAIN_OUT_FFPF: 6}.get(kind, kind)
         self._op("bc_rowchain", (kind, Cc, M, rows_per_batch, x, affine, g_tot, g_gamma, g_beta, g_groups, g_eps, res, res2, r2, r2_xmin, r2_bmod, out_w, wstream, vec, out0, out1, out2,
                                  ldvt, gn_tot, ln_eps, alpha, alpha_dev, alpha_idx, alpha_bstride, part, nsplit), "rowchain",
                  flops=2 * M * Cc * Cc * mult,
                  variant=f"rowchain_kernel<{name}{',zero' if kind in zk and out1 is not None else ''}>",
                  shape=("rowchain_" + name, M, Cc, mult * Cc), bytes_=2 * (mult * Cc * Cc + 2 * M * Cc),
-                 rocprof=f"rowchain_kernel<{Cc}, {kind}, {'true' if kind in zk and out1 is not None else 'false'}>")
+                 rocprof=f"rowchain_kernel<{Cc}, {tag}, {'true' if kind in zk and out1 is not None else 'false'}>")
         return out0
 
     def rowchain_sum(self, Cc, M, rows_per_batch, part, nsplit, out0, gn_tot=None, out1=None):
diff --git a/blobctrl_amd/weights.py b/blobctrl_amd/weights.py
--- a/blobctrl_amd/weights.py
+++ b/blobctrl_amd/weights.py
@@ -417,6 +417,14 @@
     return out
 
 
+RC_RING_FF = {320: 15, 640: 10}
+
+
+def ffp_seg_frags(C: int, nks: int) -> int:
+    ring = RC_RING_FF[C]
+    return (5 * nks + ring - 1) // ring * ring
+
+
 def pack_rowchain(pw: "PackedTrunk", p: str, kind: int, zero_name: Optional[str] = None, nsplit: int = 1):
     h, f = pw.h, pw.f
     bp = p + "transformer_blocks.0."
@@ -443,6 +451,8 @@
         bv, bg = b1[:, 0].reshape(hid), b1[:, 1].reshape(hid)
         w1o = torch.cat([wv, wg], 0)
         w2 = h[bp + "ff.net.2.weight"]
+        if kind == 7:
+            w2 = (h[p + "proj_out.weight"].float() @ w2.float()).half()
         seg_to_out = _frag_stream(h[bp + att + ".to_out.0.weight"], nC)
         ffb, chunks = [], []
         hpw = RC_HC // nw
@@ -466,16 +476,24 @@
         seg_zero = None
         if zero_name is not None:
             seg_zero = _frag_stream(h[zero_name + ".weight"], nC)
-            if kind not in (3, 6):
+            if kind not in (3, 6, 7):
                 segs.append(seg_zero)
             vec.append(f[zero_name + ".bias"])
-        if kind in (3, 6):
+        if kind in (3, 6, 7):
             nchunks = len(chunks)
             assert nchunks % nsplit == 0, (nchunks, nsplit)
             pad = torch.zeros(nw, RC_RPAD, 64, 8, dtype=torch.float16, device=seg_to_out.device)
             per = nchunks // nsplit
-            tail = ([seg_proj_out] + ([seg_zero] if seg_zero is not None else [])) if kind == 6 else []
-            slices = [torch.cat([seg_to_out] + [x for cs in chunks[z * per:(z + 1) * per] for x in cs] + tail + [pad], 1) for z in range(nsplit)]
+            slices = []
+            for z in range(nsplit):
+                head = [seg_to_out]
+                if kind == 7:
+                    head += [_frag_stream(h[p + "proj_out.weight"], nC, 32 * z * per, 32 * (z + 1) * per),
+                             pad.new_zeros(nw, ffp_seg_frags(C, per) - 5 * per, 64, 8)]
+                tail = ([seg_proj_out] if kind == 6 else []) + ([seg_zero] if kind in (6, 7) and seg_zero is not None else [])
+                slices.append(torch.cat(head + [x for cs in chunks[z * per:(z + 1) * per] for x in cs] + tail + [pad], 1))
+            if kind == 7:
+                vec[5] = h[p + "proj_out.weight"].float() @ f[bp + "ff.net.2.bias"].float() + f[p + "proj_out.bias"].float()
             return torch.stack(slices).contiguous(), torch.cat([v.reshape(-1).float() for v in vec]).contiguous()
     pad = torch.zeros(nw, RC_RPAD, 64, 8, dtype=torch.float16, device=segs[0].device)
     return torch.cat(segs + [pad], 1).contiguous(), torch.cat([v.reshape(-1).float() for v in vec]).contiguous()
diff --git a/include/blobctrl_hip.h b/include/blobctrl_hip.h
--- a/include/blobctrl_hip.h
+++ b/include/blobctrl_hip.h
@@ -186,7 +186,7 @@
 int bc_scheduler_step_single(const float* eps, float* latents, const float* coef, int* step_idx, float* hist, int B, int h, int w,
                              const float* noise, int nsteps, int third, float* eps_out, int advance, bc_stream stream);
 
-enum { BC_CHAIN_IN = 0, BC_CHAIN_MID = 1, BC_CHAIN_OUT = 2, BC_CHAIN_OUT_FF = 3, BC_CHAIN_OUT_TAIL = 4, BC_CHAIN_MIDX = 5, BC_CHAIN_OUT_FFP = 6 };
+enum { BC_CHAIN_IN = 0, BC_CHAIN_MID = 1, BC_CHAIN_OUT = 2, BC_CHAIN_OUT_FF = 3, BC_CHAIN_OUT_TAIL = 4, BC_CHAIN_MIDX = 5, BC_CHAIN_OUT_FFP = 6, BC_CHAIN_OUT_FFPF = 7 };
 int bc_rowchain_supported(int channels, int M, int rows_per_batch);
 long long bc_rowchain_stream_frags(int channels, int kind, int blobnet, int nsplit);
 int bc_rowchain(int kind, int channels, int M, int rows_per_batch, const bc_half* x, const float* affine,
```

Result: no change. 2.454 (median of 6 runs) (+0.3%).
